# iwanders/spread_spectrum_watermarking

Hardware: AMD Instinct MI355X
Metric: Mpixels/sec embed+extract (4K batch) (higher is better)
Workload: dtype f64

## Files before the change

### spread_spectrum_watermarking_amd/csrc/base_prune.hip

```cpp
#include <algorithm>
#include <cmath>

#include "dct_pair_common.hpp"
#include "dct_pair_colops.hpp"

namespace ssw {

namespace {

constexpr int BP_BINS = 2048;
constexpr int BP_THREADS = 1024;

struct BpKey {
    int ordering;
    float s[2];
    float s0[2];
    float gain;
};

__device__ inline uint32_t bp_sortable(float v) {
    const uint32_t b = __float_as_uint(v);
    return (b & 0x80000000u) ? ~b : (b | 0x80000000u);
}

__global__ __launch_bounds__(BP_THREADS) void base_prune_decide_kernel(const float* __restrict__ coef, const float* __restrict__ energy,
                                                                       unsigned W, unsigned H, BpKey kp, unsigned k,
                                                                       unsigned* __restrict__ need, unsigned long long* __restrict__ stats,
                                                                       double* __restrict__ work, double tile_flop, double tile_bytes,
                                                                       double select_bytes) {
    __shared__ unsigned hist[BP_BINS];
    __shared__ unsigned part[BP_THREADS / 64];
    __shared__ float t_sh;
    __shared__ unsigned any_sh;
    const unsigned tid = threadIdx.x, f = blockIdx.x, tiles = W / SSW_BASE_PRUNE_TILE;
    for (unsigned b = tid; b < BP_BINS; b += BP_THREADS) hist[b] = 0u;
    if (tid == 0) { t_sh = 0.0f; any_sh = 0u; }
    __syncthreads();
    const float* plane = coef + (size_t)f * W * H;
    const unsigned quads = H * (SSW_BASE_PRUNE_TILE / 4);
    for (unsigned q = tid; q < quads; q += BP_THREADS) {
        const unsigned y = q / (SSW_BASE_PRUNE_TILE / 4), x = 4 * (q % (SSW_BASE_PRUNE_TILE / 4));
        const f32x4 c = *reinterpret_cast<const f32x4*>(plane + (size_t)y * W + x);
#pragma unroll
        for (int e = 0; e < 4; ++e) {
            if (y == 0 && x + e == 0) continue;
            float key;
            if (kp.ordering == SSW_ORDER_ENERGY) key = c[e] * c[e];
            else {
                const float scaled = ((x + e) == 0 ? kp.s0[y == 0] : kp.s[y == 0]) * c[e];
                key = scaled * scaled;
            }
            atomicAdd(&hist[bp_sortable(key) >> 21], 1u);
        }
    }
    __syncthreads();
    const unsigned b0 = BP_BINS - 2 - 2 * tid;
    const unsigned h1 = hist[b0 + 1], h0 = hist[b0];
    unsigned v = h1 + h0;
#pragma unroll
    for (int o = 1; o < 64; o <<= 1) {
        const unsigned u = __shfl_up(v, o);
        if ((tid & 63u) >= (unsigned)o) v += u;
    }
    if ((tid & 63u) == 63u) part[tid >> 6] = v;
    __syncthreads();
    unsigned before = 0;
    for (unsigned wv = 0; wv < (tid >> 6); ++wv) before += part[wv];
    const unsigned incl = before + v, excl = incl - h1 - h0;
    if (excl < k && incl >= k) {
        const unsigned bin = excl + h1 >= k ? b0 + 1 : b0;
        const uint32_t sb = (uint32_t)bin << 21;
        t_sh = (sb & 0x80000000u) ? __uint_as_float(sb & 0x7FFFFFFFu) : 0.0f;
    }
    __syncthreads();
    const float T = t_sh;
    const float* e = energy + (size_t)f * W;
    unsigned* nd = need + (size_t)f * tiles;
    for (unsigned t = tid; t < tiles; t += BP_THREADS) nd[t] = t == 0 ? 1u : 0u;
    __syncthreads();
    for (unsigned x = SSW_BASE_PRUNE_TILE + tid; x < W; x += BP_THREADS) {
        const float bound = kp.gain * e[x];
        if (!(T > 1e-30f) || !(bound < T)) { nd[x / SSW_BASE_PRUNE_TILE] = 1u; any_sh = 1u; }
    }
    __syncthreads();
    if (tid == 0 && stats) {
        unsigned computed = 0;
        for (unsigned t = 0; t < tiles; ++t) computed += nd[t];
        if (work) {
            if (computed > 1) {
                atomicAdd(&work[0], (computed - 1) * tile_flop); atomicAdd(&work[1], (computed - 1) * tile_bytes);
                atomicAdd(&work[2], (computed - 1) * select_bytes);
            }
        }
        atomicAdd(&stats[0], (unsigned long long)tiles);
        atomicAdd(&stats[1], (unsigned long long)computed);
        if (any_sh) atomicAdd(&stats[2], 1ull);
    }
}

__global__ __launch_bounds__(256) void base_prune_bound_kernel(const float* __restrict__ energy, unsigned W, size_t total, float gain,
                                                               float* __restrict__ out) {
    const size_t i = blockIdx.x * (size_t)blockDim.x + threadIdx.x;
    if (i >= total) return;
    const size_t f = i / W;
    const unsigned x = (unsigned)(i - f * W), tb = x / SSW_BASE_PRUNE_TILE * SSW_BASE_PRUNE_TILE;
    out[i] = gain * energy[f * W + tb + fwd_cm128_pos(x - tb)];
}

BpKey make_key(size_t w, size_t h, int ordering) {
    float s[2][2];
    select_ortho_scales(w, h, s);
    BpKey kp;
    kp.ordering = ordering;
    kp.s[0] = s[0][0]; kp.s[1] = s[1][0];
    kp.s0[0] = s[0][1]; kp.s0[1] = s[1][1];
    kp.gain = base_prune_gain(w, h, ordering);
    return kp;
}

}

float base_prune_gain(size_t w, size_t h, int ordering) {
    if (ordering != SSW_ORDER_ENERGY && ordering != SSW_ORDER_ENERGY_ORTHOGONAL) return 0.0f;
    if (h == 0 || h >= ((size_t)1 << 17)) return 0.0f;
    double g = 4.0 * (double)h;
    if (ordering == SSW_ORDER_ENERGY_ORTHOGONAL) {
        float s[2][2];
        select_ortho_scales(w, h, s);
        double m = 0.0;
        for (int a = 0; a < 2; ++a) for (int b = 0; b < 2; ++b) m = std::max(m, (double)s[a][b]);
        g *= m * m;
    }
    g *= 1.0 + 1.0 / 32.0;
    return nextafterf((float)g, INFINITY);
}

int launch_base_prune_decide(hipStream_t st, const float* coef, const BasePrune& bp, size_t n_frames, size_t w, size_t h) {
    if (n_frames == 0) return SSW_OK;
    if (!coef || !bp.energy || !bp.need || (reinterpret_cast<uintptr_t>(coef) & 15) != 0 || w % SSW_BASE_PRUNE_TILE != 0 || w > 0xFFFFFFull || h > 0xFFFFFFull || n_frames > 0x7FFFFFFFull ||
        bp.k == 0 || bp.k > 0xFFFFFFFFull) return SSW_ERR_BAD_ARG;
    const BpKey kp = make_key(w, h, bp.ordering);
    if (!(kp.gain > 0.0f)) return SSW_ERR_BAD_ARG;
    base_prune_decide_kernel<<<(unsigned)n_frames, BP_THREADS, 0, st>>>(coef, bp.energy, (unsigned)w, (unsigned)h, kp, (unsigned)bp.k, bp.need,
                                                                       bp.stats, bp.work, bp.tile_flop, bp.tile_bytes, bp.select_bytes);
    SSW_HIP_CHECK(hipGetLastError());
    return SSW_OK;
}

int launch_base_prune_bound(hipStream_t st, const float* energy, size_t n_frames, size_t w, size_t h, int ordering, float* out) {
    const size_t total = n_frames * w;
    if (total == 0) return SSW_OK;
    if (!energy || !out || w % SSW_BASE_PRUNE_TILE != 0) return SSW_ERR_BAD_ARG;
    const float gain = base_prune_gain(w, h, ordering);
    if (!(gain > 0.0f)) return SSW_ERR_UNSUPPORTED;
    base_prune_bound_kernel<<<(unsigned)((total + 255) / 256), 256, 0, st>>>(energy, (unsigned)w, total, gain, out);
    SSW_HIP_CHECK(hipGetLastError());
    return SSW_OK;
}

}
```

### spread_spectrum_watermarking_amd/csrc/dct_pair_f64.hip

```cpp
#include "dct_pair_common.hpp"

#include <cstdlib>
#include <type_traits>

#ifdef SSW_TILE_TRACE
namespace ssw {
__device__ unsigned long long* g_tile_trace = nullptr;
__device__ unsigned int g_tile_trace_cap = 0;
__device__ unsigned int g_tile_trace_n = 0;
__device__ unsigned int* g_tile_kstep = nullptr;
extern "C" int ssw_debug_set_tile_kstep(void* dev_ptr) {
    unsigned int* p = static_cast<unsigned int*>(dev_ptr);
    return hipMemcpyToSymbol(HIP_SYMBOL(g_tile_kstep), &p, sizeof(p)) == hipSuccess ? 0 : -1;
}
extern "C" int ssw_debug_set_tile_trace(void* dev_ptr, unsigned cap) {
    unsigned long long* p = static_cast<unsigned long long*>(dev_ptr);
    unsigned zero = 0;
    if (hipMemcpyToSymbol(HIP_SYMBOL(g_tile_trace), &p, sizeof(p)) != hipSuccess) return -1;
    if (hipMemcpyToSymbol(HIP_SYMBOL(g_tile_trace_cap), &cap, sizeof(cap)) != hipSuccess) return -1;
    if (hipMemcpyToSymbol(HIP_SYMBOL(g_tile_trace_n), &zero, sizeof(zero)) != hipSuccess) return -1;
    return 0;
}
extern "C" int ssw_debug_get_tile_trace_count(unsigned* n) {
    return hipMemcpyFromSymbol(n, HIP_SYMBOL(g_tile_trace_n), sizeof(*n)) == hipSuccess ? 0 : -1;
}
}
#endif
#include "dct_pair_f64_kernel.hpp"
#if defined(SSW_TILE_TRACE) && !defined(SSW_TILE_TRACE_FWD_ONLY)
#define SSW_INV_PART -1
#include "dct_pair_f64_inv.inc"
#endif

namespace ssw {



int launch_dct_pair_gemm_multi_f64(hipStream_t st, bool is_row, bool inverse, int n_classes, const PairClassDesc* desc, float* out,
                                   double* tmp, size_t n_frames, size_t w, size_t h, Epilogue ep, const RgbSink* sink, double* tmp_out,
                                   const PairLayout& lay, const FuseCols* fuse) {
    if (n_frames == 0 || n_classes == 0) return SSW_OK;
    if (n_classes < 0 || n_classes > 8 || !desc) return SSW_ERR_BAD_ARG;
    if (w > 0xFFFFFFull || h > 0xFFFFFFull) return SSW_ERR_BAD_DIMS;
    const bool fuse_rows = fuse && fuse->mode == FUSE_ROWS_COP, fuse_cols = fuse && fuse->mode == FUSE_COLS;
    if (fuse && (!(fuse_rows || fuse_cols) || fuse_rows != is_row || inverse || w % 128 != 0 || h % 16 != 0 ||
                 pair_kpad(h / 8) != dct_pair_fused_units(h))) return SSW_ERR_BAD_ARG;
    if (fuse_rows && (!lay.class_major || sink || !fuse->cop || !fuse->rot1 || !fuse->rot2 || !fuse->rot3)) return SSW_ERR_BAD_ARG;
    const size_t lines = fuse_rows ? n_frames * 16 * dct_pair_fused_units(h) : is_row ? n_frames * h : n_frames * w;
    const size_t len = is_row ? w : h;
    if (lines > 0xFFFFFFFFull) return SSW_ERR_BAD_DIMS;
    const unsigned L = (unsigned)lines;
    const bool with_sink = sink && sink->rgb;
    PairMulti ml;
    PairInstance inst{0, false, 0};
    unsigned tiles_n = 0, leff0 = 0;
    const bool tile48 = tuning(TUNE_TILE48) != 0;
    for (int c = 0; c < n_classes; ++c) {
        PairInstance ic{0, false, 0};
        PairClassArgs& ca = ml.c[c];
        SSW_TRY(pair_class_args(desc[c].cls, is_row, inverse, len, lay, with_sink, tmp_out != nullptr, tile48, ca, ic));
        ca.x1 = desc[c].x1; ca.x2 = desc[c].x2; ca.y1 = desc[c].y1; ca.y2 = desc[c].y2;
        const unsigned ninv = inverse ? (unsigned)(len / pair_class_row(desc[c].cls).inv_ndiv) : 0u;
        if (c == 0) { inst = ic; leff0 = ninv; }
        else if (!(ic == inst) && !(ic.epi == inst.epi && ic.samex == inst.samex && n_classes > 1)) return SSW_ERR_BAD_ARG;
        if (ninv != leff0) return SSW_ERR_BAD_ARG;
        if ((unsigned long long)ml.c[c].Kp * L * 8 > 0xFFFFFFFFull) return SSW_ERR_BAD_DIMS;
        tiles_n += ml.c[c].tiles_n;
    }
    if (n_classes > 1) inst.subname = inverse ? inst.subname : 3;
    const bool small = (unsigned long long)((L + 127) / 128) * tiles_n < 448;
    if (fuse && small) return SSW_ERR_BAD_ARG;
    const int row_part = fuse_rows ? fuse->row_part : 0;
    if (row_part) {
        if ((row_part == 2 && !fuse->need) || (row_part != 1 && row_part != 2)) return SSW_ERR_BAD_ARG;
        tiles_n = 0;
        for (int c = 0; c < n_classes; ++c) {
            PairClassArgs& ca = ml.c[c];
            if (ca.tiles_n < 2 || ca.gsh > 16 || ca.bn32 == 1) return SSW_ERR_BAD_ARG;
            if (row_part == 1) ca.tiles_n = 1;
            else { ca.tn0 = 1; ca.tiles_n -= 1; }
            tiles_n += ca.tiles_n;
        }
    }
    const unsigned BM = small ? 64 : 128;
    if (small)
        for (int c = 0; c < n_classes; ++c)
            if (ml.c[c].bn32 == 2) { tiles_n -= ml.c[c].tiles_n; ml.c[c].bn32 = 0; ml.c[c].tiles_n = (ml.c[c].NP + 63) / 64; tiles_n += ml.c[c].tiles_n; }
    const bool tile0_grid = fuse_cols && fuse->tile_mode == 1;
    const unsigned tiles_m = tile0_grid ? (unsigned)n_frames : (L + BM - 1) / BM;
    if (small && n_classes == 1) {
        const int force = (int)tuning(TUNE_BN32);
        auto balance = [](unsigned long long n) { return (double)n / (256.0 * (double)((n + 255) / 256)); };
        const unsigned tn32 = (ml.c[0].NP + 31) / 32;
        const bool bn32 = force >= 0 ? force != 0 : 0.92 * balance((unsigned long long)tiles_m * tn32) > balance((unsigned long long)tiles_m * tiles_n);
        if (bn32) { ml.c[0].tiles_n = tiles_n = tn32; ml.c[0].bn32 = 1; }
    }
    const unsigned long long nblk = (unsigned long long)tiles_m * tiles_n;
    if (nblk > 0x7FFFFFFFull) return SSW_ERR_BAD_DIMS;
    ml.n_classes = (unsigned)n_classes; ml.L = L; ml.tiles_m = tiles_m; ml.tiles_n_total = tiles_n;
    PairOut po{out, tmp, (unsigned)w, (unsigned)h, (unsigned)(inverse ? leff0 : len), 0, 1, 2};
    po.tmp_out = tmp_out;
    const PairClass c0 = desc[0].cls;
    if (lay.class_major && inverse && pair_class_row(c0).split && c0 != PairClass::R2A) { po.cm = lay.rows_l2 ? 2u : 1u; po.cmt = lay.tile; }
    if (lay.class_major && inverse && c0 == PairClass::R2A) po.cm = 1;
    if (lay.class_major && inverse && is_row && lay.rows_l2 && (c0 == PairClass::E2 || c0 == PairClass::O2)) po.tcm = 1;
    if (lay.class_major && !inverse) po.ft = lay.tile;
    if (fuse_rows) {
        if (inst.samex || inst.epi != EPI_FWD || po.ft != 128) return SSW_ERR_BAD_ARG;
        po.cop = fuse->cop; po.cop_k16 = (unsigned)pair_kpad(h / 8); po.cop_lines = (unsigned)(n_frames * w);
        po.cop_hup = (unsigned)dct_pair_fused_units(h);
        po.crot1 = fuse->rot1; po.crot2 = fuse->rot2; po.crot3 = fuse->rot3;
        inst.epi = EPI_FWD_COLOP;
    }
    if (fuse_cols) po.xperm = 1;
    const bool energy = fuse_rows && fuse->energy != nullptr;
    po.col_energy = energy ? fuse->energy : nullptr;
    ml.need = nullptr; ml.need_mode = 0; ml.need_tpf = 1;
    if (fuse_cols && fuse->tile_mode) {
        if (inst.epi != EPI_FWD || inst.samex || small || (fuse->tile_mode == 2 && !fuse->need)) return SSW_ERR_BAD_ARG;
        ml.need = fuse->need; ml.need_mode = (unsigned)fuse->tile_mode; ml.need_tpf = (unsigned)(w / 128);
    }
    if (row_part == 2) {
        if (energy || po.ft != 128) return SSW_ERR_BAD_ARG;
        ml.need = fuse->need; ml.need_tpf = (unsigned)(w / 128);
        ml.tail = fuse->tail; ml.tail_flop = fuse->tail_flop; ml.tail_bytes = fuse->tail_bytes;
    }
    auto al = [](const void* p, unsigned a) { return (reinterpret_cast<uintptr_t>(p) & (a - 1)) == 0; };
    po.wide = (!is_row && w % 4 == 0 && al(out, 16) && (n_frames * w) % 4 == 0 && (!tmp || al(tmp, 16)) && (!tmp_out || al(tmp_out, 16))) ? 1u : 0u;
    if (with_sink && !(al(sink->iq_i, 16) && al(sink->iq_q, 16) && al(sink->rgb, sink->u8 ? 4 : 16))) po.wide = 0;
    if (with_sink) {
        if (is_row) return SSW_ERR_BAD_ARG;
        po.iq_i = sink->iq_i; po.iq_q = sink->iq_q; po.rgb = sink->rgb; po.rgb_u8 = sink->u8 ? 1u : 0u;
    }
    ml.po = po;
    switch (inst.epi) {
    case EPI_FWD_COLOP:
        if (row_part == 2) SSW_LAUNCH_PAIR_BM(false, EPI_FWD_COLOP, false, 5, 128);
        else if (energy) { if (inst.subname == 4) SSW_LAUNCH_PAIR_BM(false, EPI_FWD_COLOP, false, 14, 128); else SSW_LAUNCH_PAIR_BM(false, EPI_FWD_COLOP, false, 13, 128); }
        else if (inst.subname == 4) SSW_LAUNCH_PAIR_BM(false, EPI_FWD_COLOP, false, 4, 128);
        else SSW_LAUNCH_PAIR_BM(false, EPI_FWD_COLOP, false, 3, 128);
        break;
    case EPI_FWD_ADJ: SSW_LAUNCH_PAIR(false, EPI_FWD_ADJ, false); break;
    case EPI_FWD:
        if (ml.need_mode) SSW_LAUNCH_PAIR_BM(true, EPI_FWD, false, 13, 128);
        else if (inst.subname == 4) SSW_LAUNCH_PAIR_SUB(false, EPI_FWD, false, 4);
        else if (inst.subname == 3) { if (is_row) SSW_LAUNCH_PAIR_SUB(false, EPI_FWD, false, 3); else SSW_LAUNCH_PAIR_SUB(true, EPI_FWD, false, 3); }
        else if (inst.samex) SSW_LAUNCH_ROWCOL(EPI_FWD, true);
        else SSW_LAUNCH_ROWCOL(EPI_FWD, false);
        break;
    default: return launch_pair_gemm_inverse_instances(st, ml, ep, inst, is_row, small, nblk);
    }
    SSW_HIP_CHECK(hipGetLastError());
    return SSW_OK;
}

int launch_dct_pair_gemm_rows_subset_f64(hipStream_t st, const double* x, const double* y, unsigned cap, unsigned Kp, float* out,
                                         unsigned out_stride, unsigned off, size_t lines) {
    if (lines == 0 || cap == 0) return SSW_OK;
    if (lines > 0xFFFFFFFFull || (cap & 1)) return SSW_ERR_BAD_DIMS;
    const unsigned L = (unsigned)lines, NP = cap / 2;
    const unsigned tiles_m = (L + 127) / 128, tiles_n = (NP + 63) / 64;
    const unsigned long long nblk = (unsigned long long)tiles_m * tiles_n;
    if (nblk > 0x7FFFFFFFull) return SSW_ERR_BAD_DIMS;
    if ((unsigned long long)Kp * L * sizeof(double) > 0xFFFFFFFFull) return SSW_ERR_BAD_DIMS;
    PairMulti ml;
    ml.c[0] = PairClassArgs{x, x, y, y + (size_t)NP * 8, NP, Kp, cap, tiles_n, off, off + NP, 1, 0, 0xFFFFFFFFu, 0, 0, 0};
    ml.n_classes = 1; ml.L = L; ml.tiles_m = tiles_m; ml.tiles_n_total = tiles_n;
    ml.po = PairOut{out, nullptr, out_stride, 0, 0, off, off + NP, 1};
    const Epilogue ep{1.f, 1.f};
    pair_gemm_f64_kernel<false, EPI_FWD, true, 2><<<(unsigned)nblk, PT, 0, st>>>(ml, ep);
    SSW_HIP_CHECK(hipGetLastError());
    return SSW_OK;
}

int launch_dct_pair_gemm_rows_subset_split_f64(hipStream_t st, const double* x1, const double* x2, const double* y1, const double* y2,
                                               unsigned cap, unsigned Kp, float* out, unsigned out_stride, unsigned off, size_t lines) {
    if (lines == 0 || cap == 0) return SSW_OK;
    if (lines > 0xFFFFFFFFull) return SSW_ERR_BAD_DIMS;
    const unsigned L = (unsigned)lines, NP = cap;
    const unsigned tiles_m = (L + 127) / 128, tiles_n = (NP + 63) / 64;
    const unsigned long long nblk = (unsigned long long)tiles_m * tiles_n;
    if (nblk > 0x7FFFFFFFull) return SSW_ERR_BAD_DIMS;
    if ((unsigned long long)Kp * L * sizeof(double) > 0xFFFFFFFFull) return SSW_ERR_BAD_DIMS;
    PairMulti ml;
    ml.c[0] = PairClassArgs{x1, x2, y1, y2, NP, Kp, cap, tiles_n, off, 0, 1, 2, 0xFFFFFFFFu, 0, 0, 0};
    ml.n_classes = 1; ml.L = L; ml.tiles_m = tiles_m; ml.tiles_n_total = tiles_n;
    ml.po = PairOut{out, nullptr, out_stride, 0, 0, off, 0, 1};
    const Epilogue ep{1.f, 1.f};
    pair_gemm_f64_kernel<false, EPI_FWD, false, 3><<<(unsigned)nblk, PT, 0, st>>>(ml, ep);
    SSW_HIP_CHECK(hipGetLastError());
    return SSW_OK;
}

int launch_dct_pair_gemm_rows_subset_merged_f64(hipStream_t st, const PairSubsetClass* classes, unsigned n_classes, float* out,
                                                unsigned out_stride, size_t lines) {
    if (lines == 0) return SSW_OK;
    if (lines > 0xFFFFFFFFull) return SSW_ERR_BAD_DIMS;
    const unsigned L = (unsigned)lines, tiles_m = (L + 127) / 128;
    for (int split = 0; split < 2; ++split) {
        PairMulti ml;
        ml.n_classes = 0; ml.L = L; ml.tiles_m = tiles_m; ml.tiles_n_total = 0;
        auto flush = [&]() -> int {
            if (ml.n_classes == 0) return SSW_OK;
            const unsigned long long nblk = (unsigned long long)tiles_m * ml.tiles_n_total;
            if (nblk > 0x7FFFFFFFull) return SSW_ERR_BAD_DIMS;
            ml.po = PairOut{out, nullptr, out_stride, 0, 0, 0, 0, 1};
            const Epilogue ep{1.f, 1.f};
            if (split) pair_gemm_f64_kernel<false, EPI_FWD, false, 3><<<(unsigned)nblk, PT, 0, st>>>(ml, ep);
            else       pair_gemm_f64_kernel<false, EPI_FWD, true, 2><<<(unsigned)nblk, PT, 0, st>>>(ml, ep);
            SSW_HIP_CHECK(hipGetLastError());
            ml.n_classes = 0; ml.tiles_n_total = 0;
            return SSW_OK;
        };
        for (unsigned c = 0; c < n_classes; ++c) {
            const PairSubsetClass& k = classes[c];
            if ((k.x2 != nullptr) != (split != 0) || k.cap == 0) continue;
            if (!split && (k.cap & 1)) return SSW_ERR_BAD_DIMS;
            if ((unsigned long long)k.Kp * L * sizeof(double) > 0xFFFFFFFFull) return SSW_ERR_BAD_DIMS;
            const unsigned NP = split ? k.cap : k.cap / 2, tiles_n = (NP + 63) / 64;
            if (split) ml.c[ml.n_classes] = PairClassArgs{k.x1, k.x2, k.y1, k.y2, NP, k.Kp, k.cap, tiles_n, k.off, 0, 1, 2, 0xFFFFFFFFu, 0, 0, 0};
            else       ml.c[ml.n_classes] = PairClassArgs{k.x1, k.x1, k.y1, k.y1 + (size_t)NP * 8, NP, k.Kp, k.cap, tiles_n, k.off, k.off + NP, 1, 0, 0xFFFFFFFFu, 0, 0, 0};
            ml.tiles_n_total += tiles_n;
            if (++ml.n_classes == 8) SSW_TRY(flush());
        }
        SSW_TRY(flush());
    }
    return SSW_OK;
}

}
```

### spread_spectrum_watermarking_amd/csrc/dct_pair_f64_kernel.hpp

```cpp
#pragma once
#include "dct_pair_common.hpp"
#include "dct_pair_colops.hpp"

#include <cstdlib>
#include <type_traits>


namespace ssw {

constexpr int PT = 256;
constexpr int PBK = 8;
constexpr int RGB_NB = 2;

#ifdef SSW_TILE_TRACE
#define SSW_TT(i) do { if (threadIdx.x == 0) tt[i] = wall_clock64(); } while (0)
#define SSW_KT(t) do { if (threadIdx.x == 0 && (t) < 32u) kst_lds[t] = (unsigned)wall_clock64(); } while (0)
#else
#define SSW_TT(i) do { } while (0)
#define SSW_KT(t) do { } while (0)
#endif
typedef PairOutT<double> PairOut;


struct PairMulti {
    PairClassArgs c[8];
    unsigned n_classes, L, tiles_m, tiles_n_total;
    PairOut po;
    const unsigned* need = nullptr;
    unsigned need_mode = 0, need_tpf = 1;
    unsigned long long* tail = nullptr;
    double tail_flop = 0.0, tail_bytes = 0.0;
};

template <bool COLS, int EPI, bool SAMEX, int SUB = 0, int BM = 128>
__global__ __launch_bounds__(PT, 2) void pair_gemm_f64_kernel(const PairMulti ml, Epilogue ep) {
#if defined(__HIP_DEVICE_COMPILE__)
    constexpr int NX = SAMEX ? 1 : 2;
    constexpr int BN = 64, XQ = BM / 64;
    constexpr int STG = NX * BM * PBK + 2 * BN * PBK;
    constexpr int SXD = 2 * STG;
    constexpr int TRD = COLS ? 4 * 32 * (BM / 2 + 16) / 2 : 0;
#ifdef SSW_TILE_TRACE
    __shared__ __attribute__((aligned(16))) double lds[(SXD > TRD ? SXD : TRD) + 16];
    unsigned* kst_lds = reinterpret_cast<unsigned*>(lds + (SXD > TRD ? SXD : TRD));
#else
    __shared__ __attribute__((aligned(16))) double lds[SXD > TRD ? SXD : TRD];
#endif

#ifdef SSW_TILE_TRACE
    unsigned long long tt[5] = {0, 0, 0, 0, 0};
    const unsigned long long cyc0 = clock64();
    unsigned kslot = 0xFFFFFFFFu;
    if (threadIdx.x == 0 && g_tile_trace) kslot = atomicAdd(&g_tile_trace_n, 1u);
#endif
    SSW_TT(0);
    unsigned tm, tn, cls = 0;
    tile_of_block(blockIdx.x, gridDim.x, ml.tiles_m, ml.tiles_n_total, tm, tn);
    while (cls + 1 < ml.n_classes && tn >= ml.c[cls].tiles_n) { tn -= ml.c[cls].tiles_n; ++cls; }
    if constexpr (COLS && EPI == EPI_FWD && BM == 128 && SUB >= 10) {
        if (ml.need_mode == 1) tm *= ml.need_tpf;
        else if (tm % ml.need_tpf == 0 || ml.need[tm] == 0) return;
    }
    if constexpr (!COLS && EPI == EPI_FWD_COLOP && SUB == 5) {
        const PairClassArgs& cg = ml.c[cls];
        tn += cg.tn0;
        const unsigned tw = cg.bn32 == 2 ? 48u : 64u;
        const unsigned tpf = ml.po.cop_hup / 8, z = tm / tpf;
        const unsigned pf = tn * tw, pl = pf + tw - 1u < cg.NP ? pf + tw - 1u : cg.NP - 1u;
        const unsigned lo = (pf - cg.e2off) >> cg.gsh, hi = pl >> cg.gsh;
        unsigned any = 0;
        for (unsigned t = lo; t <= hi; ++t) any |= ml.need[(size_t)z * ml.need_tpf + t];
        if (!any) return;
        if (ml.tail && tm == z * tpf && threadIdx.x == 0) {
            const double pairs = (double)(pl - pf + 1u);
            atomicAdd(&ml.tail[0], 1ull);
            atomicAdd(reinterpret_cast<double*>(ml.tail) + 1, pairs * ml.tail_flop);
            atomicAdd(reinterpret_cast<double*>(ml.tail) + 2, pairs * ml.tail_bytes);
        }
    }
    const PairClassArgs& ca = ml.c[cls];
    const double* __restrict__ X1g = ca.x1;
    const double* __restrict__ X2g = ca.x2;
    const double* __restrict__ Y1g = ca.y1;
    const double* __restrict__ Y2g = ca.y2;
    const unsigned L = ml.L, NP = ca.NP, Kp = ca.Kp, yrows = ca.yrows;
    PairOut po = ml.po;
    po.c1 = ca.c1; po.c2 = ca.c2; po.cs = ca.cs; po.pm = ca.pm; po.np1 = ca.np1; po.p2lo = ca.p2lo; po.bn32 = ca.bn32; po.fold0 = ca.fold0;
    po.gsh = ca.gsh; po.e2off = ca.e2off;
    const unsigned m0 = tm * BM, p0 = tn * (po.bn32 == 1 ? 32u : po.bn32 == 2 ? 48u : (unsigned)BN);
    const unsigned tid = threadIdx.x;
    const unsigned lane = tid & 63, wave = tid >> 6;
    const unsigned li = lane & 15, lq = lane >> 4;

    const unsigned wv = (unsigned)__builtin_amdgcn_readfirstlane((int)wave);
    const unsigned drow = 16 * wave + (lane >> 2), dch = lane & 3;
    unsigned xoff[XQ];
#pragma unroll
    for (int q = 0; q < XQ; ++q) {
        const unsigned j = drow + 64 * q;
        unsigned r = m0 + ((COLS && BM == 128 && po.xperm) ? fwd_cm128_pos(j) : j);
        r = r < L ? r : L - 1;
        xoff[q] = (r - m0) * 64u + 16u * (dch ^ ((j >> 2) & 3u));
    }
    unsigned yr = p0 + drow;
    yr = yr < NP ? yr : NP - 1;
    const unsigned yoff = (yr - p0) * 64u + 16u * (dch ^ ((drow >> 2) & 3u));
#ifdef SSW_ABL_X0
    const size_t m0x = 0;
#else
    const size_t m0x = m0;
#endif
    const __amdgpu_buffer_rsrc_t x1r = __builtin_amdgcn_make_buffer_rsrc((void*)(X1g + m0x * 8), 0, 0xFFFFFFFFu, 0x00020000);
    const __amdgpu_buffer_rsrc_t x2r = __builtin_amdgcn_make_buffer_rsrc((void*)(X2g + m0x * 8), 0, 0xFFFFFFFFu, 0x00020000);
    const __amdgpu_buffer_rsrc_t y1r = __builtin_amdgcn_make_buffer_rsrc((void*)(Y1g + (size_t)p0 * 8), 0, 0xFFFFFFFFu, 0x00020000);
    const __amdgpu_buffer_rsrc_t y2r = __builtin_amdgcn_make_buffer_rsrc((void*)(Y2g + (size_t)p0 * 8), 0, 0xFFFFFFFFu, 0x00020000);
    const unsigned xstep = L * 64u, ystep = yrows * 64u;

    constexpr int LPT = XQ * NX + 2;
    typedef __attribute__((address_space(3))) void* lds_ptr_t;
    auto issue = [&](unsigned t, unsigned sb) {
        const unsigned xadv = t * xstep, yadv = t * ystep;
        double* b = lds + sb + 16 * wv * PBK;
#pragma unroll
        for (int q = 0; q < XQ; ++q) {
            __builtin_amdgcn_raw_ptr_buffer_load_lds(x1r, (lds_ptr_t)(b + 64 * q * PBK), 16, xoff[q], xadv, 0, 0);
            if (!SAMEX) __builtin_amdgcn_raw_ptr_buffer_load_lds(x2r, (lds_ptr_t)(b + BM * PBK + 64 * q * PBK), 16, xoff[q], xadv, 0, 0);
        }
        __builtin_amdgcn_raw_ptr_buffer_load_lds(y1r, (lds_ptr_t)(b + NX * BM * PBK), 16, yoff, yadv, 0, 0);
        __builtin_amdgcn_raw_ptr_buffer_load_lds(y2r, (lds_ptr_t)(b + NX * BM * PBK + BN * PBK), 16, yoff, yadv, 0, 0);
    };
    auto run = [&](auto nic, auto njc) {
    constexpr int NI = decltype(nic)::value;
    constexpr int NJ = decltype(njc)::value;
    constexpr int NJA = NJ < 2 ? 2 : NJ;
    constexpr bool FULL = NI == BM / 32;
    const unsigned wm = FULL ? (wave >> 1) * (BM / 2) : wave * (BM / 4), wn = FULL ? (wave & 1) * 32 : 0;
    f64x4 acc1[NI][NJA], acc2[NI][NJA];
#pragma unroll
    for (int i = 0; i < NI; ++i)
#pragma unroll
        for (int j = 0; j < NJA; ++j) { acc1[i][j] = (f64x4){0, 0, 0, 0}; acc2[i][j] = (f64x4){0, 0, 0, 0}; }

    const unsigned fsw = (li >> 2) & 3;
    unsigned rdx[2], rdy[2];
#pragma unroll
    for (int sh = 0; sh < 2; ++sh) {
        rdx[sh] = (wm + li) * PBK + 2 * ((2 * sh + (lq >> 1)) ^ fsw) + (lq & 1);
        rdy[sh] = NX * BM * PBK + (wn + li) * PBK + 2 * ((2 * sh + (lq >> 1)) ^ fsw) + (lq & 1);
    }
    struct Frag { double x1[NI], x2[NI], y1[NJA], y2[NJA]; };
    auto fread = [&](unsigned sb, auto shc, Frag& f) {
        constexpr int sh = decltype(shc)::value;
        const double* b = lds + sb;
#pragma unroll
        for (int jn = 0; jn < NJ; ++jn) {
            f.y1[jn] = b[rdy[sh] + 16 * jn * PBK];
            f.y2[jn] = b[rdy[sh] + BN * PBK + 16 * jn * PBK];
        }
#pragma unroll
        for (int i = 0; i < NI; ++i) {
            f.x1[i] = b[rdx[sh] + 16 * i * PBK];
            if (!SAMEX) f.x2[i] = b[rdx[sh] + BM * PBK + 16 * i * PBK];
        }
    };
    auto fmma = [&](const Frag& f) {
#pragma unroll
        for (int i = 0; i < NI; ++i)
#pragma unroll
            for (int jn = 0; jn < NJ; ++jn) {
                const double xb = SAMEX ? f.x1[i] : f.x2[i];
                if (!COLS) {
                    acc1[i][jn] = __builtin_amdgcn_mfma_f64_16x16x4f64(f.x1[i], f.y1[jn], acc1[i][jn], 0, 0, 0);
                    acc2[i][jn] = __builtin_amdgcn_mfma_f64_16x16x4f64(xb, f.y2[jn], acc2[i][jn], 0, 0, 0);
                } else {
                    acc1[i][jn] = __builtin_amdgcn_mfma_f64_16x16x4f64(f.y1[jn], f.x1[i], acc1[i][jn], 0, 0, 0);
                    acc2[i][jn] = __builtin_amdgcn_mfma_f64_16x16x4f64(f.y2[jn], xb, acc2[i][jn], 0, 0, 0);
                }
            }
    };
    using B0 = std::integral_constant<int, 0>;
    using B1 = std::integral_constant<int, 1>;
    auto interleave = [&](auto dmac) {
        constexpr int NDMA = decltype(dmac)::value;
        constexpr int NMF = 2 * NJ * NI;
        constexpr int NRD = (2 * NJ + NI * NX + 1) / 2;
#pragma unroll
        for (int i = 0; i < NRD; ++i) {
            __builtin_amdgcn_sched_group_barrier(0x008, 1, 0);
            __builtin_amdgcn_sched_group_barrier(0x100, 1, 0);
        }
#pragma unroll
        for (int i = 0; i < NDMA; ++i) {
            __builtin_amdgcn_sched_group_barrier(0x008, 1, 0);
            __builtin_amdgcn_sched_group_barrier(0x020, 1, 0);
        }
        __builtin_amdgcn_sched_group_barrier(0x008, NMF - NRD - NDMA > 0 ? NMF - NRD - NDMA : 0, 0);
        __builtin_amdgcn_sched_barrier(0);
    };
    const unsigned nk = Kp / PBK;
    Frag fa, fb;
    issue(0, 0);
    issue(1, STG);
    asm volatile("s_waitcnt vmcnt(%0)" :: "n"(LPT) : "memory");
    asm volatile("s_barrier" ::: "memory");
    SSW_TT(1);
    fread(0u, B0{}, fa);
    unsigned cur = 0, nxt = STG, t = 0;
    auto step = [&](auto issuec) {
        constexpr bool ISSUE = decltype(issuec)::value != 0;
        fread(cur, B1{}, fb);
        fmma(fa);
        interleave(B0{});
        asm volatile("s_waitcnt vmcnt(0) lgkmcnt(0)\n\ts_barrier" ::: "memory");
// ... 597 lines not shown
                        const unsigned ln = m0 + wm + 16 * i + li;
                        const unsigned lz = ln < L ? ln / W : 0, lc = ln < L ? ln - lz * W : 0;
                        const double* tp = po.tmp + (size_t)lz * (n / 2) * W + lc;
#pragma unroll
                        for (int r = 0; r < 4; ++r) {
                            const unsigned pair = p0 + wn + 16 * jn + lq + 4 * r;
                            const unsigned pc = pair < NP ? pair : 0;
                            const unsigned nn = half ? po.c2 + po.cs * p2(pc) : po.c1 + po.cs * pc;
                            e[i][r] = tp[(size_t)(nn < n / 2 ? nn : 0) * W];
                        }
                    }
                    (void)tpl;
                    lds_order();
#pragma unroll
                    for (int i = 0; i < NI; ++i)
#pragma unroll
                        for (int r = 0; r < 4; ++r) {
                            const double a = half ? acc2[i][jn][r] : acc1[i][jn][r];
                            tw[wr0 + (4 * r) * TPF + 16 * i] = (float)(e[i][r] + a);
                            tw[wr0 + (16 + 4 * r) * TPF + 16 * i] = (float)(e[i][r] - a);
                        }
                    lds_order();
                    if constexpr (EPI == EPI_INV_O_RGB) {
                        if (rgb_fast) {
                            auto rgb_round = [&](auto u8c) {
                            constexpr bool U8 = decltype(u8c)::value;
                            constexpr int NB = NRI < RGB_NB ? NRI : RGB_NB;
#pragma unroll
                            for (int tb = 0; tb < NRI; tb += NB) {
                                unsigned off[NB];
                                float fac[NB];
                                f32x4 v[NB], iv[NB], qv[NB];
#pragma unroll
                                for (int u = 0; u < NB; ++u) {
                                    const int t = tb + u;
                                    const unsigned srow = t * RPI + rrow;
                                    const unsigned pair = p0 + wn + 16 * jn + (srow & 15);
                                    v[u] = *reinterpret_cast<const f32x4*>(trd + t * RPI * TPF);
                                    const unsigned pc = pair < NP ? pair : 0;
                                    const unsigned nn = half ? po.c2 + po.cs * p2(pc) : po.c1 + po.cs * pc;
                                    const bool ok = line_ok && pair < NP && nn < n / 2;
                                    const unsigned idx = srow < 16 ? nn : n - 1 - nn;
                                    off[u] = ok ? idx * W + col : 0x20000000u;
                                    fac[u] = idx == 0 ? ep.first : ep.base;
                                    iv[u] = __builtin_bit_cast(f32x4, __builtin_amdgcn_raw_buffer_load_b128(rgb_i, off[u] * 4u, 0, 0));
                                    qv[u] = __builtin_bit_cast(f32x4, __builtin_amdgcn_raw_buffer_load_b128(rgb_q, off[u] * 4u, 0, 0));
                                }
#pragma unroll
                                for (int u = 0; u < NB; ++u) {
                                    float y[4], c[12];
#pragma unroll
                                    for (int e4 = 0; e4 < 4; ++e4) y[e4] = plain ? v[u][e4] : v[u][e4] * fac[u];
                                    pair_rgb_of_quad(y, iv[u], qv[u], c);
                                    if (U8) {
                                        unsigned w3[3];
                                        pair_rgb8_words(c, w3);
                                        __builtin_amdgcn_raw_buffer_store_b96((u32x3){w3[0], w3[1], w3[2]}, rgb_o, off[u] * 3u, 0, 0);
                                    } else {
#pragma unroll
                                        for (int d = 0; d < 3; ++d)
                                            __builtin_amdgcn_raw_buffer_store_b128(__builtin_bit_cast(u32x4, (f32x4){c[4 * d], c[4 * d + 1], c[4 * d + 2], c[4 * d + 3]}),
                                                                                   rgb_o, off[u] * 12u + 16u * d, 0, 0);
                                    }
                                }
                            }
                            };
                            if (po.rgb_u8) rgb_round(std::true_type{}); else rgb_round(std::false_type{});
                            continue;
                        }
                    }
#pragma unroll
                    for (int t = 0; t < NRI; ++t) {
                        const unsigned srow = t * RPI + rrow;
                        const unsigned pair = p0 + wn + 16 * jn + (srow & 15);
                        const f32x4 v = *reinterpret_cast<const f32x4*>(trd + t * RPI * TPF);
                        if (!line_ok || pair >= NP) continue;
                        const unsigned nn = half ? po.c2 + po.cs * p2(pair) : po.c1 + po.cs * pair;
                        if (nn >= n / 2) continue;
                        put_quad(srow < 16 ? nn : n - 1 - nn, v);
                    }
                }
        }
        trace_end();
        return;
      }
    }
    if constexpr (COLS) {
#pragma unroll
        for (int i = 0; i < NI; ++i) {
            const unsigned line = m0 + wm + 16 * i + li;
            if (line >= L) continue;
            const unsigned z = line / W, col = line - z * W;
            float* lp = po.out + (size_t)z * H * W + col;
            double* tp = po.tmp + (size_t)z * (n / 2) * W + col;
            if (EPI == EPI_INV_O_RGB) {
                const size_t base = (size_t)z * H * W + col;
#pragma unroll
                for (int jn = 0; jn < NJ; ++jn)
#pragma unroll
                    for (int r = 0; r < 4; r += 2) {
                        double e1[2], e2[2];
                        bool ok1[2], ok2[2];
                        unsigned m1[2], m2[2];
#pragma unroll
                        for (int q = 0; q < 2; ++q) {
                            const unsigned pair = p0 + wn + 16 * jn + lq + 4 * (r + q);
                            const unsigned pc = pair < NP ? pair : 0;
                            const unsigned n1 = po.c1 + po.cs * pc, n2 = po.c2 + po.cs * p2(pc);
                            ok1[q] = pair < NP && n1 < n / 2;
                            ok2[q] = pair < NP && n2 < n / 2;
                            m1[q] = ok1[q] ? n1 : 0;
                            m2[q] = ok2[q] ? n2 : 0;
                            e1[q] = tp[(size_t)m1[q] * W];
                            e2[q] = tp[(size_t)m2[q] * W];
                        }
#pragma unroll
                        for (int q = 0; q < 2; ++q) {
                            const double a1 = acc1[i][jn][r + q], a2 = acc2[i][jn][r + q];
                            const unsigned idx1[2] = {m1[q], n - 1 - m1[q]}, idx2[2] = {m2[q], n - 1 - m2[q]};
                            const float v1[2] = {(float)(e1[q] + a1), (float)(e1[q] - a1)}, v2[2] = {(float)(e2[q] + a2), (float)(e2[q] - a2)};
                            unsigned px1[2], px2[2];
                            float y1[2], y2[2];
#pragma unroll
                            for (int o = 0; o < 2; ++o) {
                                px1[o] = idx1[o] * W; y1[o] = apply_epilogue(ep, v1[o], idx1[o]);
                                px2[o] = idx2[o] * W; y2[o] = apply_epilogue(ep, v2[o], idx2[o]);
                            }
                            pair_store_rgb_batch<double, 2>(po, base, px1, y1, ok1[q]);
                            pair_store_rgb_batch<double, 2>(po, base, px2, y2, ok2[q]);
                        }
                    }
                continue;
            }
#pragma unroll
            for (int jn = 0; jn < NJ; ++jn)
#pragma unroll
                for (int r = 0; r < 4; ++r) {
                    const unsigned pair = p0 + wn + 16 * jn + lq + 4 * r;
                    if (pair >= NP) continue;
                    emit(lp, tp, po.tmp_out + (size_t)z * n * W + col, W, pair, acc1[i][jn][r], acc2[i][jn][r]);
                }
        }
    }
    trace_end();
    };
    using J1 = std::integral_constant<int, 1>;
    using J2 = std::integral_constant<int, 2>;
    using J3 = std::integral_constant<int, 3>;
    const bool j3 = BM == 128 && (po.bn32 == 2 || (!COLS && NP - p0 <= 48));
    if (NP - p0 <= 16 && po.bn32 != 2) run(std::integral_constant<int, BM / 64>{}, J1{});
    else if (po.bn32 != 2 && (NP - p0 <= 32 || po.bn32)) run(std::integral_constant<int, BM / 64>{}, J2{});
    else if (j3)                       run(std::integral_constant<int, BM / 64>{}, J3{});
    else                               run(std::integral_constant<int, BM / 32>{}, J2{});
#endif
}

#define SSW_LAUNCH_PAIR_BM(COLS, EPI, SAMEX, SUBV, BMV) \
        pair_gemm_f64_kernel<COLS, EPI, SAMEX, SUBV, BMV><<<(unsigned)nblk, PT, 0, st>>>(ml, ep)
#define SSW_LAUNCH_PAIR_SUB(COLS, EPI, SAMEX, SUBV) do { if (small) SSW_LAUNCH_PAIR_BM(COLS, EPI, SAMEX, SUBV, 64); else SSW_LAUNCH_PAIR_BM(COLS, EPI, SAMEX, SUBV, 128); } while (0)
#define SSW_LAUNCH_PAIR(COLS, EPI, SAMEX) do { if (inst.subname == 0) SSW_LAUNCH_PAIR_SUB(COLS, EPI, SAMEX, 0); else SSW_LAUNCH_PAIR_SUB(COLS, EPI, SAMEX, 1); } while (0)
#define SSW_LAUNCH_ROWCOL(EPI, SAMEX) do { if (is_row) SSW_LAUNCH_PAIR(false, EPI, SAMEX); else SSW_LAUNCH_PAIR(true, EPI, SAMEX); } while (0)

int launch_pair_gemm_inverse_instances(hipStream_t st, const PairMulti& ml, Epilogue ep, const PairInstance& inst, bool is_row, bool small,
                                       unsigned long long nblk);

}
```

### spread_spectrum_watermarking_amd/csrc/ssw_internal.hpp

```cpp
#pragma once

#include <hip/hip_runtime.h>

#include <cstddef>
#include <cstdint>
#include <functional>
#include <map>
#include <string>
#include <tuple>
#include <utility>
#include <vector>

#include "../../include/ssw.h"
#include "dct_plan.hpp"
#include "dct_pair_class.hpp"

namespace ssw {

void set_last_error(const std::string& s);

#define SSW_HIP_CHECK(expr)                                                              \
    do {                                                                                 \
        hipError_t e__ = (expr);                                                         \
        if (e__ != hipSuccess) {                                                         \
            ::ssw::set_last_error(std::string(#expr) + ": " + hipGetErrorString(e__));   \
            return (e__ == hipErrorOutOfMemory) ? SSW_ERR_OUT_OF_MEMORY : SSW_ERR_HIP;   \
        }                                                                                \
    } while (0)

#define SSW_TRY(expr)                         \
    do {                                      \
        int s__ = (expr);                     \
        if (s__ != SSW_OK) return s__;        \
    } while (0)


int launch_rgb_to_yiq(hipStream_t st, const float* rgb, size_t npix, float* y, float* i, float* q);
int launch_yiq_to_rgb(hipStream_t st, const float* y, const float* i, const float* q, size_t npix,
                      float* rgb);
int launch_synth(hipStream_t st, uint32_t seed, uint32_t first_frame, size_t n_frames, size_t w,
                 size_t h, float* rgb);

size_t dense_basis_kpad(size_t n);
int launch_make_basis_f32(hipStream_t st, size_t n, bool inverse, float* out);
int launch_make_basis_f64(hipStream_t st, size_t n, bool inverse, double* out);

struct Epilogue {
    float first, base;
};
int launch_dct_rows(hipStream_t st, int precision, const float* in, float* out, size_t rows, size_t w,
                    const void* basis, Epilogue ep);
int launch_dct_cols(hipStream_t st, int precision, const float* in, float* out, size_t n_frames,
                    size_t w, size_t h, const void* basis, Epilogue ep);
int launch_dct_rows_f64out(hipStream_t st, const float* in, double* out, size_t rows, size_t w, const double* basis);
int launch_dct_cols_f64out(hipStream_t st, const float* in, double* out, size_t n_frames, size_t w, size_t h, const double* basis);

size_t dct_pair_kpad(size_t n);
size_t dct_pair_operand_elems(size_t n_frames, size_t w, size_t h);
int launch_make_half_basis_blocked(hipStream_t st, size_t n, bool inverse, int parity, double* out);
int launch_dct_pair_prep(hipStream_t st, bool is_row, bool inverse, const float* in, size_t n_frames, size_t w, size_t h,
                         double* o1, double* o2);
enum class PixFmt { F32, U8, U16 };
constexpr size_t pix_bytes(PixFmt f) { return f == PixFmt::U8 ? 1 : f == PixFmt::U16 ? 2 : 4; }
constexpr unsigned pix_align_mask(PixFmt f) { return f == PixFmt::U8 ? 3u : f == PixFmt::U16 ? 7u : 15u; }
bool dct_pair_can_prep_from_rgb(size_t w, size_t h, const void* rgb, PixFmt fmt);
enum class RowSrc { Plane, RgbF32, RgbU8, RgbU16 };
constexpr RowSrc row_src(PixFmt f) { return f == PixFmt::U8 ? RowSrc::RgbU8 : f == PixFmt::U16 ? RowSrc::RgbU16 : RowSrc::RgbF32; }
constexpr PixFmt pix_fmt(RowSrc s) { return s == RowSrc::RgbU8 ? PixFmt::U8 : s == RowSrc::RgbU16 ? PixFmt::U16 : PixFmt::F32; }
struct RowInput {
    RowSrc kind; const void* p; float *i, *q;
    static RowInput plane(const float* y) { return {RowSrc::Plane, y, nullptr, nullptr}; }
    static RowInput rgb(PixFmt f, const void* frames, float* i = nullptr, float* q = nullptr) { return {row_src(f), frames, i, q}; }
};
int launch_dct_pair_prep4(hipStream_t st, bool is_row, bool inverse, const RowInput& in, size_t n_frames, size_t w, size_t h,
                          double* q1, double* q2, double* p);
int launch_dct_pair_prep8_rows(hipStream_t st, const RowInput& in, size_t n_frames, size_t w, size_t h,
                               double* r1, double* r2, double* m, double* p);
struct RgbSink {
    const float* iq_i = nullptr;
    const float* iq_q = nullptr;
    void* rgb = nullptr;
    bool u8 = false;
};
int launch_dct_pair_prep8_cols(hipStream_t st, const float* in, size_t n_frames, size_t w, size_t h,
                               double* r1, double* r2, double* m, double* p);
enum { FUSE_ROWS_COP = 1, FUSE_COLS = 2 };
struct FuseCols {
    int mode = 0; double* cop = nullptr; const double *rot1 = nullptr, *rot2 = nullptr, *rot3 = nullptr;
    float* energy = nullptr;
    const unsigned* need = nullptr;
    int tile_mode = 0;
    int row_part = 0;
    unsigned long long* tail = nullptr;
    double tail_flop = 0.0, tail_bytes = 0.0;
};
struct PairClassDesc { PairClass cls; const double *x1, *x2, *y1, *y2; };
int launch_dct_pair_gemm_multi_f64(hipStream_t st, bool is_row, bool inverse, int n_classes, const PairClassDesc* desc, float* out,
                                   double* tmp, size_t n_frames, size_t w, size_t h, Epilogue ep, const RgbSink* sink = nullptr,
                                   double* tmp_out = nullptr, const PairLayout& layout = PairLayout(), const FuseCols* fuse = nullptr);

int launch_dct_pair_gemm_rows_subset_f64(hipStream_t st, const double* x, const double* y, unsigned cap, unsigned Kp, float* out,
                                         unsigned out_stride, unsigned off, size_t lines);
int launch_dct_pair_gemm_rows_subset_split_f64(hipStream_t st, const double* x1, const double* x2, const double* y1, const double* y2,
                                               unsigned cap, unsigned Kp, float* out, unsigned out_stride, unsigned off, size_t lines);
struct PairSubsetClass {
    const double *x1, *x2, *y1, *y2;
    unsigned cap, Kp, off;
};
int launch_dct_pair_gemm_rows_subset_merged_f64(hipStream_t st, const PairSubsetClass* classes, unsigned n_classes, float* out,
                                                unsigned out_stride, size_t lines);
size_t dct_pair_split_kpad(size_t len);
enum { TUNE_EFOLD_MIN, TUNE_EFOLD_INV_MIN, TUNE_EFOLD_COLS_MIN, TUNE_CLASS_TILE, TUNE_DEEP_MIN_ROWS, TUNE_DEEP_MIN_COLS, TUNE_PREP_STAGED,
       TUNE_MERGE_MAX_LINES, TUNE_BN32, TUNE_BAND_SPLIT, TUNE_FUSE_COLS, TUNE_UPLOAD_BANDS, TUNE_SPECULATE_K, TUNE_PREP_LIGHT, TUNE_LANE_STAGGER, TUNE_DERIVED_FUSED, TUNE_TILE48, TUNE_BASE_PRUNE, TUNE_BASE_ENERGY_LOWP, TUNE_COUNT };
long long tuning(int which);
int launch_prep16_cols_l2(hipStream_t st, const float* in, size_t n_frames, size_t w, size_t h, double* base,
                          const double* rot1, const double* rot2, const double* rot3, bool class_major, bool in_l2, unsigned K16);
int launch_prep16_inv_cols_l2(hipStream_t st, const float* in, size_t n_frames, size_t w, size_t h, double* base,
                              const double* rot1, const double* rot2, const double* rot3, bool class_major, bool in_l2, unsigned K16);
int launch_prep16_cols_staged(hipStream_t st, const float* in, size_t n_frames, size_t w, size_t h, double* base,
                              const double* rot1, const double* rot2, bool class_major, bool semi, unsigned K8, unsigned K16, bool efold);
int launch_prep16_inv_cols_staged(hipStream_t st, const float* in, size_t n_frames, size_t w, size_t h, double* base,
                                  const double* rot1, const double* rot2, bool class_major, bool semi, unsigned K8, unsigned K16, bool l2);
int launch_prep16_inv_rows_l2(hipStream_t st, const float* in, size_t rows, size_t w, double* base,
                              const double* rot1, const double* rot2, const double* rot3, unsigned K16);
int launch_prep16_inv_rows_staged(hipStream_t st, const float* in, size_t rows, size_t w, double* base,
                                  const double* rot1, const double* rot2, unsigned K8, unsigned K16);
size_t dct_pair_split_elems(size_t n_frames, size_t w, size_t h);
size_t dct_pair_split_basis_rows(size_t len, int which);
int launch_make_split_basis_blocked(hipStream_t st, size_t n, bool inverse, int which, double* out);
int launch_make_rot_table(hipStream_t st, size_t n, double* out);
int launch_dct_pair_rotate(hipStream_t st, const double* p, const double* rot, double* sp, size_t lines, size_t len);
size_t dct_pair_semi_deep_elems(size_t lines, size_t len);
int launch_dct_pair_prep16_inv_rows(hipStream_t st, const float* in, size_t n_frames, size_t w, size_t h, double* base,
                                    const double* rot1, const double* rot2, const double* rot3, PrepFamily prep);
int launch_dct_pair_prep16_inv_cols(hipStream_t st, const float* in, size_t n_frames, size_t w, size_t h, double* base,
                                    const double* rot1, const double* rot2, const double* rot3, PrepFamily prep, const PairLayout& lay);
int launch_dct_pair_prep16_cols(hipStream_t st, const float* in, size_t n_frames, size_t w, size_t h, double* base,
                                const double* rot1, const double* rot2, const double* rot3, PrepFamily prep, const PairLayout& lay);
size_t dct_pair_deep_elems(size_t lines, size_t len);
int launch_dct_pair_prep16_rows(hipStream_t st, const RowInput& in, size_t n_frames, size_t w, size_t h, double* base,
                                const double* rot1, const double* rot2, const double* rot3, bool l2, bool unit_order = false);
inline size_t dct_pair_fused_units(size_t h) { return ((h / 16 + 7) / 8) * 8; }

constexpr unsigned PRUNE_NO_REM = 0xFFFFFFFFu;
constexpr uint32_t PRUNE_NEG = 0x40000000u;
constexpr unsigned SSW_PRUNE_INFO = 16;
struct PruneClass { unsigned mod, rem, cap, off, rem2 = PRUNE_NO_REM, radd = 0; };
struct PrunePlan {
    unsigned n_classes = 0;
    PruneClass c[9];
    unsigned W = 0, cap_total = 0;
};
static_assert(SSW_PRUNE_INFO >= 1 + sizeof(PrunePlan::c) / sizeof(PruneClass), "a chunk's info block holds the flag and one count per class");
int launch_prune_build(hipStream_t st, const uint32_t* idx, size_t n_frames, size_t k, const PrunePlan& plan,
                       uint32_t* flag , uint32_t* rows , uint32_t* pos , uint32_t* info );
struct PruneGatherJob {
    const uint32_t* rows;
    const char* src;
    char* dst;
    unsigned cap, src_rows, kblocks, first_block;
    bool negate;
    bool frag = false;
};
struct PruneGatherJobs {
    PruneGatherJob j[18];
    unsigned n;
};
int launch_prune_gather_bases(hipStream_t st, PruneGatherJobs jobs);
int launch_extract_pruned(hipStream_t st, const float* base, const float* compact, size_t n_frames, size_t w, size_t h,
                          size_t cap, const uint32_t* pos, const uint32_t* indices, size_t k, int method, float alpha,
                          float* out);

constexpr unsigned SSW_BASE_PRUNE_TILE = 128;
constexpr unsigned SSW_BASE_PRUNE_STATS = 16;
struct BasePrune {
    float* energy = nullptr;
    unsigned* need = nullptr;
    unsigned long long* stats = nullptr;
    size_t k = 0;
    int ordering = 0;
    double* work = nullptr;
    double tile_flop = 0.0, tile_bytes = 0.0, select_bytes = 0.0;
    bool* decided = nullptr;
    std::function<int(hipStream_t)>* tail = nullptr;
};
float base_prune_gain(size_t w, size_t h, int ordering);
int launch_base_prune_decide(hipStream_t st, const float* coef, const BasePrune& bp, size_t n_frames, size_t w, size_t h);
int launch_base_prune_bound(hipStream_t st, const float* energy, size_t n_frames, size_t w, size_t h, int ordering, float* out);

struct BaseEnergyClass {
    const double *x1 = nullptr, *x2 = nullptr;
    const void* y16 = nullptr;
    unsigned NP = 0, Kp = 0, pair0 = 0, pm = 0, c1 = 0, c2 = 0, gsh = 0, e2off = 0;
};
size_t base_energy_split_bytes(unsigned NP, unsigned Kp, unsigned pair0);
int launch_base_energy_split(hipStream_t st, const double* y1, const double* y2, unsigned yrows, unsigned NP, unsigned Kp, unsigned pair0, void* out);
int launch_base_energy_bound(hipStream_t st, int n_classes, const BaseEnergyClass* cls, size_t n_frames, size_t w, size_t h, size_t lines_per_frame,
                             float factor, float* energy);

struct SelectWorkspace {
    uint32_t* hist = nullptr;
    uint32_t* ctrl = nullptr;
    uint64_t* cand = nullptr;
    size_t frames = 0, cap = 0;
    uint32_t* fallbacks = nullptr;
};
size_t select_cand_capacity(size_t k);
size_t select_max_k();
void select_ortho_scales(size_t w, size_t h, float s[2][2]);
int launch_topk(hipStream_t st, const float* coef, size_t n_frames, size_t w, size_t h, int ordering,
                size_t k, const SelectWorkspace& ws, uint32_t* indices, const unsigned* need = nullptr, unsigned need_tile = 0,
                size_t cand_cap = 0);
struct ResizeTaps {
    uint32_t max_taps = 0;
    std::vector<uint32_t> left, count;
    std::vector<float> weights;
};
struct DeviceTaps {
    uint32_t* left = nullptr;
    uint32_t* count = nullptr;
    float* weights = nullptr;
    uint32_t max_taps = 0;
    uint32_t span[8] = {0};
    bool quad_uniform = false;
};
void build_resize_taps(size_t in_len, size_t out_len, ResizeTaps& t);
int launch_u8_to_f32(hipStream_t st, const uint8_t* in, size_t n, float* out);
int launch_f32_to_u8(hipStream_t st, const float* in, size_t n, uint8_t* out);
int launch_rgb8_to_yiq(hipStream_t st, const uint8_t* rgb, size_t npix, float* y, float* i, float* q);
int launch_u16_to_f32(hipStream_t st, const uint16_t* in, size_t n, float* out);
int launch_f32_to_u16(hipStream_t st, const float* in, size_t n, uint16_t* out);
int launch_rgb16_to_yiq(hipStream_t st, const uint16_t* rgb, size_t npix, float* y, float* i, float* q);
int launch_yiq_to_rgb8(hipStream_t st, const float* y, const float* i, const float* q, size_t npix, uint8_t* rgb);
size_t resize_tmp_bytes(const uint8_t* in, size_t n_frames, size_t w, size_t h, size_t nw, size_t nh, const DeviceTaps& vt,
                        const DeviceTaps& ht, const uint8_t* out);
int launch_resize_rgb8(hipStream_t st, const uint8_t* in, size_t n_frames, size_t w, size_t h, size_t nw, size_t nh,
                       const DeviceTaps& vt, const DeviceTaps& ht, float* tmp, uint8_t* out);

int full_sort_scratch_bytes(size_t plane_len, size_t n_frames, size_t* bytes);
int launch_full_sort(hipStream_t st, const float* coef, size_t n_frames, size_t w, size_t h, int ordering, void* scratch,
                     size_t scratch_bytes, uint32_t* indices_out, size_t k);
int launch_embed(hipStream_t st, float* coef, size_t n_frames, size_t plane_len,
                 const uint32_t* indices, size_t idx_stride, const float* marks,
                 const uint32_t* mark_offsets, const uint32_t* mark_lens, size_t n_marks,
                 size_t max_len, size_t mark_stride , int method, float alpha);
int launch_extract(hipStream_t st, const float* base, const float* derived, size_t n_frames,
                   size_t plane_len, const uint32_t* indices, size_t k, int method, float alpha,
                   float* out);
int launch_similarity(hipStream_t st, const float* extracted, const float* marks, size_t n_pairs,
                      size_t k, float* sims);
int launch_extract_shared(hipStream_t st, const float* base, const float* derived, size_t n_frames, size_t plane_len,
                          const uint32_t* indices, size_t k, int method, float alpha, float* out);
int launch_extract_shared_pruned(hipStream_t st, const float* base, const float* compact, size_t n_frames, size_t w, size_t h,
                                 size_t cap, const uint32_t* pos, const uint32_t* indices, size_t k, int method, float alpha,
                                 float* out);
int launch_trace_finish(hipStream_t st, const float* sims, size_t n_rows, size_t n_marks, float threshold, const float* extracted,
                        const float* marks, size_t k, uint32_t* best, float* best_sim, uint32_t* n_exceed);
int launch_gemm_nt_f32(hipStream_t st, const float* A, size_t M, const float* B, size_t N, size_t K, float* out);
int launch_sim_den(hipStream_t st, const float* extracted, size_t n_ext, size_t k, float* den);
int launch_sim_scale(hipStream_t st, float* sims, const float* den, size_t n_ext, size_t n_marks);
int launch_widen_indices(hipStream_t st, const uint32_t* in, size_t n, uint64_t* out);

}

namespace ssw { namespace host { struct Transfer; } }

struct ssw_ctx {
    int device = 0;
    hipStream_t stream = nullptr;
    hipStream_t own_stream = nullptr;
    size_t chunk_frames = 0;

    std::map<std::tuple<size_t, bool, bool, ssw::BasisKind>, void*> basis;
    std::map<std::tuple<size_t, int, unsigned>, void*> split16;
    bool fold = true;
    int fold_level = SSW_DCT_FOLDING_DEFAULT;

    struct Buf {
        void* p = nullptr;
        size_t bytes = 0;
    };
    struct Lane {
        Buf plane[4];
        Buf operand[6];
        Buf idx;
        ssw::SelectWorkspace sel;
        Buf compact[2];
        Buf gathered;
        Buf prune_u32;
        Buf base_prune;
        hipStream_t cur = nullptr;
        hipEvent_t done = nullptr;
    };
    static constexpr int MAX_LANES = 2;
    Lane lane[MAX_LANES];
    hipStream_t aux_stream = nullptr;
    bool overlap = true;
    bool prune = true;
    bool split = true;
    std::vector<hipEvent_t> sync_events;
    size_t sync_next = 0;
    Buf overflow;
    uint64_t pruned_chunks = 0, redone_chunks = 0;
    uint64_t pruned_columns = 0;
    Buf base_prune_stats;
    double base_prune_billed[5] = {0.0, 0.0, 0.0, 0.0, 0.0};
    hipStream_t copy_stream = nullptr;
    struct FrameStage {
        Buf buf;
        static constexpr int MAX_BANDS = 4;
        hipEvent_t uploaded[MAX_BANDS] = {nullptr, nullptr, nullptr, nullptr};
        hipEvent_t consumed = nullptr;
        bool in_use = false;
    };
    FrameStage frame_stage[2];
    unsigned frame_stage_next = 0;
    size_t expected_k = 0;
    std::multimap<size_t, void*> plane_pool;
    size_t plane_pool_bytes = 0;
    struct RgbSpare { void* p; size_t bytes; hipEvent_t released; };
    std::vector<RgbSpare> rgb_spares;
    std::vector<void*> retired;
    uint32_t* select_fallbacks = nullptr;
    uint64_t select_frames = 0;
    ssw::host::Transfer* xfer = nullptr;
    hipStream_t down_stream = nullptr;
    struct HostStream {
        static constexpr int NB = 3;
        Buf in[NB], in2[NB], out[NB];
        Buf marks, ext, sims;
        hipEvent_t up_done[NB] = {}, k_done[NB] = {}, down_done[NB] = {};
        bool active = false;
    };
    HostStream hs;
    Buf small;
    Buf sort_scratch;
    Buf resize_tmp;
    Buf restore_base;
    Buf trace[6];
    Buf locate[6];
    Buf catalogue[3];
    Buf jpeg;
    Buf filter;
    Buf fingerprint[6];
    std::map<std::pair<size_t, size_t>, ssw::DeviceTaps> taps;

    bool timing = false;
    double stage_ms[SSW_STAGE_COUNT] = {0};
    uint64_t stage_launches[SSW_STAGE_COUNT] = {0};
    double stage_bytes[SSW_STAGE_COUNT] = {0};
    double stage_work[SSW_STAGE_COUNT] = {0};
    struct Pending {
        int stage;
        hipEvent_t a, b;
        int alias = -1;
    };
    std::vector<Pending> pending;
    std::vector<hipEvent_t> free_events;
    hipEvent_t tail_event = nullptr;
    hipStream_t tail_stream = nullptr;
    bool tail_fresh = false;
};
namespace ssw { inline PlanSettings plan_settings(const ssw_ctx* ctx) { return PlanSettings{ctx->fold, ctx->fold_level, ctx->split}; } }
```

### spread_spectrum_watermarking_amd/csrc/ssw_lib.hip

```cpp
#include <algorithm>
#include <cmath>
#include <cstdlib>
#include <cstring>
#include <new>

#include "resize_common.hpp"
#include "ssw_host.hpp"

namespace ssw {
static thread_local std::string g_last_error;
void set_last_error(const std::string& s) { g_last_error = s; }
}

using namespace ssw;
using namespace ssw::host;

struct ssw_writer {
    ssw_ctx* ctx;
    size_t w, h;
    ssw_config cfg;
    float *y = nullptr, *i = nullptr, *q = nullptr;
    float* y0 = nullptr;
    uint32_t* idx = nullptr;
    size_t idx_k = 0;
// ... 102 lines not shown
    {
        ssw_ctx::FrameStage& fs = ctx->frame_stage[ctx->frame_stage_next & 1];
        SSW_TRY(grow(fs.buf, bytes));
        const bool no_split = tuning(TUNE_BAND_SPLIT) == 0;
        long long nb = tuning(TUNE_UPLOAD_BANDS);
        nb = nb < 2 ? 2 : nb > ssw_ctx::FrameStage::MAX_BANDS ? ssw_ctx::FrameStage::MAX_BANDS : nb;
        while (nb > 2 && ((bytes / nb) % 16 != 0 || !can_split_forward_rows(ctx, precision == SSW_PRECISION_F64, w, h, (size_t)nb, y, tmp, fs.buf.p, fmt))) --nb;
        if (!no_split && bytes >= ((size_t)8 << 20) &&
            can_split_forward_rows(ctx, precision == SSW_PRECISION_F64, w, h, (size_t)nb, y, tmp, fs.buf.p, fmt)) {
            ++ctx->frame_stage_next;
            SSW_TRY(frame_stage_events(fs));
            if (fs.in_use) SSW_HIP_CHECK(hipStreamWaitEvent(ctx->copy_stream, fs.consumed, 0));
            const size_t hb = bytes / nb, hp = plane / nb, rows = h / nb;
            bool in_flight = false;
            int rc = SSW_OK;
            for (int band = 0; band < (int)nb && rc == SSW_OK; ++band) {
                bool async = false;
                rc = upload_nowait(ctx, (char*)fs.buf.p + band * hb, (const char*)host_rgb + band * hb, hb, ctx->copy_stream, &async);
                in_flight = in_flight || async;
                if (rc == SSW_OK && hipEventRecord(fs.uploaded[band], ctx->copy_stream) != hipSuccess) rc = SSW_ERR_HIP;
                if (rc == SSW_OK && hipStreamWaitEvent(ctx->stream, fs.uploaded[band], 0) != hipSuccess) rc = SSW_ERR_HIP;
                untimed_work(ctx);
                if (rc != SSW_OK) break;
                Chain ch;
                rc = build_forward_rows_band(ctx, ctx->lane[0], precision, (char*)fs.buf.p + band * hb, fmt, w, rows, h, tmp + band * hp,
                                             i ? i + band * hp : nullptr, q ? q + band * hp : nullptr, ch);
                if (rc == SSW_OK) rc = run_serial(ch, ctx->stream);
            }
            if (rc == SSW_OK) rc = stage_consumed(ctx, fs);
            if (rc == SSW_OK) {
                Chain ch;
                rc = build_forward_cols_after_rows(ctx, ctx->lane[0], precision, w, h, tmp, y, ch);
                if (rc == SSW_OK) rc = run_serial(ch, ctx->stream);
            }
            if (in_flight && hipStreamSynchronize(ctx->copy_stream) != hipSuccess && rc == SSW_OK) rc = SSW_ERR_HIP;
            return rc;
        }
    }
    ssw_ctx::FrameStage* fs = nullptr;
    SSW_TRY(stage_frame_in(ctx, host_rgb, bytes, &fs));
    Chain ch;
    SSW_TRY(build_forward_from_rgb(ctx, ctx->lane[0], precision, fs->buf.p, fmt, 1, w, h, y, i, q, tmp, ch));
    SSW_TRY(run_serial(ch, ctx->stream));
    return stage_consumed(ctx, *fs);
}
int similarity_matrix_enqueue(ssw_ctx* ctx, const float* dev_extracted, size_t n_extracted, const float* dev_marks, size_t n_marks,
                              size_t k, float* dev_sims) {
    SSW_TRY(grow(ctx->small, n_extracted * sizeof(float)));
    StageTimer t(ctx, SSW_STAGE_SIMILARITY, ctx->stream);
    SSW_TRY(launch_sim_den(ctx->stream, dev_extracted, n_extracted, k, (float*)ctx->small.p));
    SSW_TRY(launch_gemm_nt_f32(ctx->stream, dev_extracted, n_extracted, dev_marks, n_marks, k, dev_sims));
    return launch_sim_scale(ctx->stream, dev_sims, (const float*)ctx->small.p, n_extracted, n_marks);
}
}

namespace ssw {
namespace host {
int trace_check_args(const ssw_ctx* ctx, const ssw_config* cfg, size_t w, size_t h, size_t k, const void* marks, size_t n_marks,
                     const void* sims, const void* best, const void* best_sim, const void* n_exceed) {
    if (!ctx) return SSW_ERR_BAD_ARG;
    if (!marks && (n_marks || sims || best || best_sim || n_exceed)) return SSW_ERR_BAD_ARG;
    SSW_TRY(check_config(cfg));
    if (w == 0 || h == 0) return SSW_ERR_BAD_DIMS;
    if (k >= w * h) return SSW_ERR_K_TOO_LARGE;
    return SSW_OK;
}

int trace_score(ssw_ctx* ctx, const float* dev_extracted, size_t n_suspects, const float* dev_marks, size_t n_marks, size_t k,
                float threshold, float* dev_sims, uint32_t* dev_best, float* dev_best_sim, uint32_t* dev_n_exceed) {
    if (n_suspects == 0 || (!dev_sims && !dev_best && !dev_best_sim && !dev_n_exceed)) return SSW_OK;
    float* sims = dev_sims;
    if (!sims && n_marks) {
        SSW_TRY(grow(ctx->trace[5], n_suspects * n_marks * sizeof(float)));
        sims = (float*)ctx->trace[5].p;
    }
    if (n_marks && k) SSW_TRY(similarity_matrix_enqueue(ctx, dev_extracted, n_suspects, dev_marks, n_marks, k, sims));
    else if (n_marks) { SSW_HIP_CHECK(hipMemsetAsync(sims, 0xFF, n_suspects * n_marks * sizeof(float), ctx->stream)); untimed_work(ctx); }
    StageTimer t(ctx, SSW_STAGE_SIMILARITY, ctx->stream);
    return launch_trace_finish(ctx->stream, sims, n_suspects, k ? n_marks : 0, threshold, dev_extracted, dev_marks, k, dev_best, dev_best_sim,
                               dev_n_exceed);
}
}
}

namespace {
int fingerprint_trace_impl(ssw_ctx* ctx, const ssw_config* cfg, const void* dev_base_rgb, const void* dev_suspect_rgb, PixFmt fmt,
                           size_t n_suspects, size_t w, size_t h, size_t k, const float* dev_marks, size_t n_marks, float threshold,
                           float* dev_extracted, float* dev_sims, uint32_t* dev_best, float* dev_best_sim, uint32_t* dev_n_exceed) {
    if (!ctx || !dev_base_rgb || !dev_suspect_rgb || !dev_extracted) return SSW_ERR_BAD_ARG;
    SSW_TRY(trace_check_args(ctx, cfg, w, h, k, dev_marks, n_marks, dev_sims, dev_best, dev_best_sim, dev_n_exceed));
    if (n_suspects == 0) return SSW_OK;
    CtxGuard g(ctx);
    const float* yb = nullptr;
    const uint32_t* idx = nullptr;
    SSW_TRY(trace_base(ctx, *cfg, dev_base_rgb, fmt, w, h, k, &yb, &idx));
    SSW_TRY(trace_extract(ctx, *cfg, yb, idx, dev_suspect_rgb, fmt, n_suspects, w, h, k, dev_extracted));
    return trace_score(ctx, dev_extracted, n_suspects, dev_marks, n_marks, k, threshold, dev_sims, dev_best, dev_best_sim, dev_n_exceed);
}
}

extern "C" {

const char* ssw_version(void) { return "ssw-hip 0.1.0 (gfx950)"; }
int ssw_build_all_strategies(void) { return 0; }

int ssw_ctx_transform_plan(ssw_ctx* ctx, size_t n_frames, size_t w, size_t h, int dct_type, uint32_t* flags) {
    if (!ctx || !flags || w == 0 || h == 0) return SSW_ERR_BAD_ARG;
    const ssw::PlanSettings s = ssw::plan_settings(ctx);
    *flags = ssw::plan_flags(ssw::plan_transform({dct_type, SSW_PRECISION_F64, std::min(n_frames, ssw::plan_frame_limit(s, true, w, h)), w, h,
                                                  0, false, true, s}));
    return SSW_OK;
}

const char* ssw_status_string(int s) {
    switch (s) {
    case SSW_OK: return "ok";
    case SSW_ERR_BAD_ARG: return "bad argument";
    case SSW_ERR_BAD_DIMS: return "bad dimensions";
    case SSW_ERR_LENGTH_MISMATCH: return "Derived coefficient length not equal to base coefficient length.";
    case SSW_ERR_K_TOO_LARGE: return "Desired extraction length exceeds available coefficients.";
    case SSW_ERR_NOT_BASE: return "reader was not created as a base reader";
    case SSW_ERR_UNSUPPORTED: return "unsupported (custom closures cannot run on the device)";
    case SSW_ERR_CONSUMED: return "writer already consumed";
    case SSW_ERR_HIP: return "HIP runtime error";
    case SSW_ERR_NO_DEVICE: return "no HIP device (this library has no CPU path)";
    case SSW_ERR_OUT_OF_MEMORY: return "out of device memory";
    default: return "unknown status";
    }
}

const char* ssw_last_error(void) { return g_last_error.c_str(); }

void ssw_config_default(ssw_config* cfg) {
    if (!cfg) return;
    cfg->ordering = SSW_ORDER_ENERGY;
    cfg->method = SSW_OPTION2;
    cfg->alpha = 0.1f;
    cfg->precision = SSW_PRECISION_F64;
}

int ssw_ctx_create(int device_id, ssw_ctx** out) {
    if (!out) return SSW_ERR_BAD_ARG;
    *out = nullptr;
    int count = 0;
    if (hipGetDeviceCount(&count) != hipSuccess || count <= 0) {
        set_last_error("hipGetDeviceCount: no device");
        return SSW_ERR_NO_DEVICE;
    }
    if (device_id < 0 || device_id >= count) return SSW_ERR_BAD_ARG;
    DeviceGuard g(device_id);
    ssw_ctx* ctx = new (std::nothrow) ssw_ctx();
    if (!ctx) return SSW_ERR_OUT_OF_MEMORY;
    ctx->device = device_id;
    hipError_t e = hipStreamCreateWithFlags(&ctx->own_stream, hipStreamNonBlocking);
    if (e != hipSuccess) { delete ctx; set_last_error(hipGetErrorString(e)); return SSW_ERR_HIP; }
    ctx->stream = ctx->own_stream;
    e = hipStreamCreateWithFlags(&ctx->aux_stream, hipStreamNonBlocking);
    if (e != hipSuccess) { (void)hipStreamDestroy(ctx->own_stream); delete ctx; set_last_error(hipGetErrorString(e)); return SSW_ERR_HIP; }
    e = hipStreamCreateWithFlags(&ctx->copy_stream, hipStreamNonBlocking);
    if (e != hipSuccess) {
        (void)hipStreamDestroy(ctx->aux_stream); (void)hipStreamDestroy(ctx->own_stream);
        delete ctx; set_last_error(hipGetErrorString(e)); return SSW_ERR_HIP;
    }
    if (hipMalloc((void**)&ctx->select_fallbacks, sizeof(uint32_t)) != hipSuccess ||
        hipMemset(ctx->select_fallbacks, 0, sizeof(uint32_t)) != hipSuccess) {
        (void)hipGetLastError();
        if (ctx->select_fallbacks) (void)hipFree(ctx->select_fallbacks);
        (void)hipStreamDestroy(ctx->copy_stream); (void)hipStreamDestroy(ctx->aux_stream); (void)hipStreamDestroy(ctx->own_stream);
        delete ctx; set_last_error("hipMalloc: selection counter"); return SSW_ERR_OUT_OF_MEMORY;
    }
    const char* ov = std::getenv("SSW_OVERLAP");
    if (ov) ctx->overlap = std::atoi(ov) != 0;
    const char* pr = std::getenv("SSW_PRUNE");
    if (pr) ctx->prune = std::atoi(pr) != 0;
    const char* sp = std::getenv("SSW_ODD_SPLIT");
    if (sp) ctx->split = std::atoi(sp) != 0;
    *out = ctx;
    return SSW_OK;
}

int ssw_ctx_destroy(ssw_ctx* ctx) {
    if (!ctx) return SSW_OK;
    CtxGuard g(ctx);
    (void)hipStreamSynchronize(ctx->stream);
    if (ctx->aux_stream) (void)hipStreamSynchronize(ctx->aux_stream);
    if (ctx->copy_stream) (void)hipStreamSynchronize(ctx->copy_stream);
    if (ctx->down_stream) (void)hipStreamSynchronize(ctx->down_stream);
    transfer_destroy(ctx);
    for (int s = 0; s < ssw_ctx::HostStream::NB; ++s) {
        release(ctx->hs.in[s]); release(ctx->hs.in2[s]); release(ctx->hs.out[s]);
        for (hipEvent_t e : {ctx->hs.up_done[s], ctx->hs.k_done[s], ctx->hs.down_done[s]}) if (e) (void)hipEventDestroy(e);
    }
    release(ctx->hs.marks); release(ctx->hs.ext); release(ctx->hs.sims);
    for (void* p : ctx->retired) (void)hipFree(p);
    ctx->retired.clear();
    (void)plane_pool_flush(ctx);
    for (auto& fs : ctx->frame_stage) {
        release(fs.buf);
        for (hipEvent_t e : fs.uploaded)
            if (e) (void)hipEventDestroy(e);
        if (fs.consumed) (void)hipEventDestroy(fs.consumed);
    }
    for (auto& kv : ctx->basis) (void)hipFree(kv.second);
    for (auto& kv : ctx->split16) (void)hipFree(kv.second);
    for (auto& ln : ctx->lane) {
        for (auto& b : ln.plane) release(b);
        for (auto& b : ln.operand) release(b);
        for (auto& b : ln.compact) release(b);
        release(ln.idx);
        release(ln.gathered);
        release(ln.prune_u32);
        release(ln.base_prune);
        release_select(ln.sel);
    }
    if (ctx->select_fallbacks) (void)hipFree(ctx->select_fallbacks);
    release(ctx->overflow);
    release(ctx->base_prune_stats);
    release(ctx->small);
    release(ctx->sort_scratch);
    release(ctx->resize_tmp);
    release(ctx->restore_base);
    for (auto& b : ctx->fingerprint) release(b);
    for (auto& b : ctx->trace) release(b);
    for (auto& b : ctx->locate) release(b);
    for (auto& b : ctx->catalogue) release(b);
    release(ctx->jpeg);
    release(ctx->filter);
    for (auto& kv : ctx->taps) { (void)hipFree(kv.second.left); (void)hipFree(kv.second.count); (void)hipFree(kv.second.weights); }
    for (auto& e : ctx->sync_events) (void)hipEventDestroy(e);
    for (auto& p : ctx->pending) { (void)hipEventDestroy(p.a); (void)hipEventDestroy(p.b); }
    for (auto& e : ctx->free_events) (void)hipEventDestroy(e);
    if (ctx->aux_stream) (void)hipStreamDestroy(ctx->aux_stream);
    if (ctx->copy_stream) (void)hipStreamDestroy(ctx->copy_stream);
    if (ctx->down_stream) (void)hipStreamDestroy(ctx->down_stream);
    (void)hipStreamDestroy(ctx->own_stream);
    delete ctx;
    return SSW_OK;
}

int ssw_ctx_synchronize(ssw_ctx* ctx) {
    if (!ctx) return SSW_ERR_BAD_ARG;
    CtxGuard g(ctx);
    SSW_HIP_CHECK(hipStreamSynchronize(ctx->stream));
    return SSW_OK;
}

void* ssw_ctx_stream(ssw_ctx* ctx) { return ctx ? (void*)ctx->stream : nullptr; }

int ssw_ctx_set_stream(ssw_ctx* ctx, void* hip_stream) {
    if (!ctx) return SSW_ERR_BAD_ARG;
    CtxGuard g(ctx);
    SSW_TRY(flush_timers(ctx));
    SSW_HIP_CHECK(hipStreamSynchronize(ctx->stream));
    ctx->stream = hip_stream ? (hipStream_t)hip_stream : ctx->own_stream;
    return SSW_OK;
}

int ssw_ctx_wait_event(ssw_ctx* ctx, void* hip_event) {
    if (!ctx || !hip_event) return SSW_ERR_BAD_ARG;
    CtxGuard g(ctx);
    SSW_HIP_CHECK(hipStreamWaitEvent(ctx->stream, (hipEvent_t)hip_event, 0));
    return SSW_OK;
}

int ssw_ctx_record_event(ssw_ctx* ctx, void* hip_event) {
    if (!ctx || !hip_event) return SSW_ERR_BAD_ARG;
    CtxGuard g(ctx);
    SSW_HIP_CHECK(hipEventRecord((hipEvent_t)hip_event, ctx->stream));
    return SSW_OK;
}

int ssw_ctx_set_chunk_frames(ssw_ctx* ctx, size_t frames) {
    if (!ctx) return SSW_ERR_BAD_ARG;
    ctx->chunk_frames = frames;
    return SSW_OK;
}

size_t ssw_ctx_pass_frames(ssw_ctx* ctx, size_t n_frames, size_t w, size_t h) {
    return ctx ? effective_chunk(ctx, w, h, n_frames) : 0;
}

int ssw_ctx_set_dct_folding(ssw_ctx* ctx, int enable) {
    if (!ctx) return SSW_ERR_BAD_ARG;
    if (enable < 0 || enable > 6) return SSW_ERR_BAD_ARG;
    ctx->fold = enable != 0;
    ctx->fold_level = enable;
    return SSW_OK;
}

int ssw_ctx_enable_timing(ssw_ctx* ctx, int enable) {
    if (!ctx) return SSW_ERR_BAD_ARG;
    CtxGuard g(ctx);
    SSW_TRY(flush_timers(ctx));
    ctx->timing = enable != 0;
    return SSW_OK;
}

int ssw_ctx_reset_timing(ssw_ctx* ctx) {
    if (!ctx) return SSW_ERR_BAD_ARG;
    CtxGuard g(ctx);
    SSW_TRY(flush_timers(ctx));
    for (int s = 0; s < SSW_STAGE_COUNT; ++s) { ctx->stage_ms[s] = 0; ctx->stage_launches[s] = 0; ctx->stage_work[s] = 0; ctx->stage_bytes[s] = 0; }
    ctx->pruned_chunks = ctx->redone_chunks = ctx->pruned_columns = 0;
    ctx->select_frames = 0;
    SSW_HIP_CHECK(hipStreamSynchronize(ctx->stream));
    if (ctx->aux_stream) SSW_HIP_CHECK(hipStreamSynchronize(ctx->aux_stream));
    SSW_HIP_CHECK(hipMemset(ctx->select_fallbacks, 0, sizeof(uint32_t)));
// ... 889 lines not shown
```

### spread_spectrum_watermarking_amd/csrc/ssw_pipeline.hip

```cpp
#include <algorithm>
#include <cmath>
#include <cstring>

#include "ssw_host.hpp"
#include "dct_pair_split.hpp"

#include <array>
#include <cstdlib>

namespace ssw {
namespace host {

namespace { thread_local ssw_ctx* tl_ctx = nullptr; }
CtxGuard::CtxGuard(ssw_ctx* ctx) : dg(ctx->device), prev(tl_ctx) {
    tl_ctx = ctx;
    if (prev != ctx) { ctx->tail_event = nullptr; ctx->tail_fresh = false; }
    if (prev != ctx && !ctx->retired.empty()) {
        for (void* p : ctx->retired) (void)hipFree(p);
        ctx->retired.clear();
    }
}
CtxGuard::~CtxGuard() { tl_ctx = prev; }

size_t plane_pool_flush(ssw_ctx* ctx) {
    size_t bytes = ctx->plane_pool_bytes;
    for (auto& kv : ctx->plane_pool) (void)hipFree(kv.second);
    ctx->plane_pool.clear();
    ctx->plane_pool_bytes = 0;
    for (auto& sp : ctx->rgb_spares) { (void)hipFree(sp.p); (void)hipEventDestroy(sp.released); bytes += sp.bytes; }
    ctx->rgb_spares.clear();
    return bytes;
}

size_t host_stream_release(ssw_ctx* ctx) {
    ssw_ctx::HostStream& hs = ctx->hs;
    if (hs.active) return 0;
    size_t bytes = 0;
    for (int s = 0; s < ssw_ctx::HostStream::NB; ++s)
        for (ssw_ctx::Buf* b : {&hs.in[s], &hs.in2[s], &hs.out[s]})
            if (b->p) { bytes += b->bytes; (void)hipFree(b->p); b->p = nullptr; b->bytes = 0; }
    return bytes;
}

int dev_malloc(void** p, size_t bytes) {
    *p = nullptr;
    hipError_t e = hipMalloc(p, bytes ? bytes : 16);
    if (e == hipSuccess) return SSW_OK;
    (void)hipGetLastError();
    if (tl_ctx && (!tl_ctx->plane_pool.empty() || !tl_ctx->rgb_spares.empty())) {
        (void)plane_pool_flush(tl_ctx);
        e = hipMalloc(p, bytes ? bytes : 16);
        if (e == hipSuccess) return SSW_OK;
        (void)hipGetLastError();
    }
    if (tl_ctx && host_stream_release(tl_ctx)) {
        e = hipMalloc(p, bytes ? bytes : 16);
        if (e == hipSuccess) return SSW_OK;
        (void)hipGetLastError();
    }
    *p = nullptr;
    set_last_error(std::string("hipMalloc(") + std::to_string(bytes) + " bytes): " + hipGetErrorString(e));
    return SSW_ERR_OUT_OF_MEMORY;
}

int grow(ssw_ctx::Buf& b, size_t bytes) {
    if (b.bytes >= bytes && b.p) return SSW_OK;
    if (b.p) {
        if (tl_ctx) tl_ctx->retired.push_back(b.p);
        else SSW_HIP_CHECK(hipFree(b.p));
        b.p = nullptr; b.bytes = 0;
    }
    SSW_ALLOC(&b.p, bytes);
    b.bytes = bytes ? bytes : 16;
    return SSW_OK;
}

void release(ssw_ctx::Buf& b) {
    if (b.p) (void)hipFree(b.p);
    b.p = nullptr;
    b.bytes = 0;
}

void release_select(SelectWorkspace& s) {
    if (s.hist) (void)hipFree(s.hist);
    if (s.ctrl) (void)hipFree(s.ctrl);
    if (s.cand) (void)hipFree(s.cand);
    s = SelectWorkspace();
}

int grow_select(hipStream_t st, SelectWorkspace& s, size_t frames, size_t k) {
    const size_t want = select_cand_capacity(k);
    if (s.frames >= frames && s.cap >= want && s.hist) return SSW_OK;
    const size_t nf = std::max(frames, s.frames), cap = std::max(want, s.cap);
    release_select(s);
    SSW_ALLOC(&s.hist, nf * 2048 * sizeof(uint32_t));
    SSW_ALLOC(&s.ctrl, nf * 4 * sizeof(uint32_t));
    SSW_ALLOC(&s.cand, nf * cap * sizeof(uint64_t));
    SSW_HIP_CHECK(hipMemsetAsync(s.hist, 0, nf * 2048 * sizeof(uint32_t), st));
    SSW_HIP_CHECK(hipMemsetAsync(s.ctrl, 0, nf * 4 * sizeof(uint32_t), st));
    untimed_work(tl_ctx);
    s.frames = nf;
    s.cap = cap;
    return SSW_OK;
}

static hipEvent_t timer_event(ssw_ctx* ctx, hipStream_t st) {
    if (ctx->tail_event && ctx->tail_fresh && ctx->tail_stream == st) return ctx->tail_event;
    hipEvent_t e = nullptr;
    if (!ctx->free_events.empty()) { e = ctx->free_events.back(); ctx->free_events.pop_back(); }
    else if (hipEventCreateWithFlags(&e, hipEventReleaseToDevice) != hipSuccess) return nullptr;
    if (hipEventRecord(e, st) != hipSuccess) { ctx->free_events.push_back(e); return nullptr; }
    ctx->tail_event = e; ctx->tail_stream = st; ctx->tail_fresh = true;
    return e;
}
StageTimer::StageTimer(ssw_ctx* c, int s, hipStream_t stream, double work, int alias_stage) : ctx(c), stage(s), st(stream), alias(alias_stage) {
    if (!ctx->timing) return;
    ctx->stage_work[stage] += work;
    if (alias >= 0) ctx->stage_work[alias] += work;
    const bool gemm = stage == SSW_STAGE_DCT_ROW || stage == SSW_STAGE_DCT_COL || stage == SSW_STAGE_DCT_ROW_MAIN || stage == SSW_STAGE_DCT_COL_MAIN;
    if (!gemm) ctx->stage_bytes[stage] += work;
    a = timer_event(ctx, st);
    ctx->tail_fresh = false;
    armed = a != nullptr;
}
void StageTimer::traffic(double bytes) {
    if (ctx->timing) ctx->stage_bytes[stage] += bytes;
}
StageTimer::~StageTimer() {
    if (!ctx->timing || !armed) return;
    b = timer_event(ctx, st);
    if (b) ctx->pending.push_back({stage, a, b, alias});
}

int flush_timers(ssw_ctx* ctx) {
    std::vector<hipEvent_t> used;
    for (auto& p : ctx->pending) {
        float ms = 0.f;
        SSW_HIP_CHECK(hipEventSynchronize(p.b));
        SSW_HIP_CHECK(hipEventElapsedTime(&ms, p.a, p.b));
        ctx->stage_ms[p.stage] += ms;
        ctx->stage_launches[p.stage] += 1;
        if (p.alias >= 0) { ctx->stage_ms[p.alias] += ms; ctx->stage_launches[p.alias] += 1; }
        used.push_back(p.a);
        used.push_back(p.b);
    }
    ctx->pending.clear();
    std::sort(used.begin(), used.end());
    used.erase(std::unique(used.begin(), used.end()), used.end());
    for (hipEvent_t e : used) ctx->free_events.push_back(e);
    ctx->tail_event = nullptr; ctx->tail_fresh = false;
    if (ctx->base_prune_stats.p) {
        double wk[3] = {0.0, 0.0, 0.0};
        SSW_HIP_CHECK(hipMemcpy(wk, (const char*)ctx->base_prune_stats.p + 4 * sizeof(unsigned long long), sizeof(wk), hipMemcpyDeviceToHost));
        if (ctx->timing) {
            ctx->stage_work[SSW_STAGE_DCT_COL] += wk[0] - ctx->base_prune_billed[0];
            ctx->stage_bytes[SSW_STAGE_DCT_COL] += wk[1] - ctx->base_prune_billed[1];
            ctx->stage_work[SSW_STAGE_SELECT] += wk[2] - ctx->base_prune_billed[2];
            ctx->stage_bytes[SSW_STAGE_SELECT] += wk[2] - ctx->base_prune_billed[2];
        }
        for (int i = 0; i < 3; ++i) ctx->base_prune_billed[i] = wk[i];
        double tw[2] = {0.0, 0.0};
        SSW_HIP_CHECK(hipMemcpy(tw, (const char*)ctx->base_prune_stats.p + 9 * sizeof(unsigned long long), sizeof(tw), hipMemcpyDeviceToHost));
        if (ctx->timing) {
            ctx->stage_work[SSW_STAGE_DCT_ROW] += tw[0] - ctx->base_prune_billed[3];
            ctx->stage_bytes[SSW_STAGE_DCT_ROW] += tw[1] - ctx->base_prune_billed[4];
        }
        for (int i = 0; i < 2; ++i) ctx->base_prune_billed[3 + i] = tw[i];
    }
    return SSW_OK;
}

int get_basis(ssw_ctx* ctx, size_t n, bool inverse, bool f64, BasisKind kind, const void** out) {
    typedef BasisKind B;
    auto key = std::make_tuple(n, inverse, f64, kind);
    auto it = ctx->basis.find(key);
    if (it != ctx->basis.end()) { *out = it->second; return SSW_OK; }
    void* p = nullptr;
    if (kind != B::Dense && !f64) return SSW_ERR_BAD_ARG;
    const bool half = kind == B::HalfEven || kind == B::HalfOdd, rot = kind == B::Rot;
    const int split_which = kind == B::SinELaunch ? 4 : (int)kind - (int)B::CosE;
    const size_t elems = kind == B::Dense ? n * dense_basis_kpad(n)
                       : rot  ? n / 2
                       : half ? (n / 2) * dct_pair_kpad(n)
                              : dct_pair_split_basis_rows(n, split_which) * dct_pair_split_kpad(n);
    SSW_ALLOC(&p, std::max<size_t>(elems, 1) * (f64 ? sizeof(double) : sizeof(float)));
    int rc = rot  ? launch_make_rot_table(ctx->stream, n, (double*)p)
             : half ? launch_make_half_basis_blocked(ctx->stream, n, inverse, kind == B::HalfOdd ? 1 : 0, (double*)p)
             : kind != B::Dense ? launch_make_split_basis_blocked(ctx->stream, n, inverse, split_which, (double*)p)
             : f64  ? launch_make_basis_f64(ctx->stream, n, inverse, (double*)p)
                    : launch_make_basis_f32(ctx->stream, n, inverse, (float*)p);
    untimed_work(ctx);
    if (rc != SSW_OK) { (void)hipFree(p); return rc; }
    ctx->basis[key] = p;
    *out = p;
    return SSW_OK;
}

int get_split16(ssw_ctx* ctx, size_t len, PairClass c, const double* y1, const double* y2, const PairClassArgs& ca, unsigned pair0, const void** out) {
    auto key = std::make_tuple(len, (int)c, pair0);
    auto it = ctx->split16.find(key);
    if (it != ctx->split16.end()) { *out = it->second; return SSW_OK; }
    void* p = nullptr;
    SSW_ALLOC(&p, base_energy_split_bytes(ca.NP, ca.Kp, pair0));
    const int rc = launch_base_energy_split(ctx->stream, y1, y2, ca.yrows, ca.NP, ca.Kp, pair0, p);
    untimed_work(ctx);
    if (rc != SSW_OK) { (void)hipFree(p); return rc; }
    ctx->split16[key] = p;
    *out = p;
    return SSW_OK;
}

bool valid_method(int m) { return m == SSW_OPTION1 || m == SSW_OPTION2 || m == SSW_OPTION3; }
bool valid_ordering(int o) { return o == SSW_ORDER_ENERGY || o == SSW_ORDER_ENERGY_ORTHOGONAL || o == SSW_ORDER_LEGACY; }
bool valid_precision(int p) { return p == SSW_PRECISION_F32 || p == SSW_PRECISION_F64; }

int check_config(const ssw_config* cfg) {
    if (!cfg) return SSW_ERR_BAD_ARG;
    if (cfg->method == SSW_METHOD_CUSTOM || cfg->ordering == SSW_ORDER_CUSTOM) return SSW_ERR_UNSUPPORTED;
    if (!valid_method(cfg->method) || !valid_ordering(cfg->ordering) || !valid_precision(cfg->precision))
        return SSW_ERR_BAD_ARG;
    return SSW_OK;
}

namespace {
size_t lane_bytes_held(const ssw_ctx* ctx) {
    size_t held = 0;
    for (const auto& ln : ctx->lane) {
        for (const auto& b : ln.plane) held += b.bytes;
        for (const auto& b : ln.operand) held += b.bytes;
        for (const auto& b : ln.compact) held += b.bytes;
        held += ln.idx.bytes + ln.gathered.bytes + ln.prune_u32.bytes;
    }
    return held;
}
}

size_t effective_chunk(const ssw_ctx* ctx, size_t w, size_t h, size_t n_frames) {
    size_t c = ctx->chunk_frames;
    if (c == 0) {
        const size_t px = std::max<size_t>(w * h, 1);
        c = std::max<size_t>(1, ((size_t)1 << 30) / px);
        const size_t per_frame = dct_pair_operand_elems(1, w, h) * sizeof(double);
        if (per_frame) c = std::max<size_t>(1, std::min(c, (size_t)0xFFFFFFFFull / per_frame));
        if (c >= 16) c &= ~(size_t)7;
        c = std::min(c, std::max<size_t>(n_frames, 1));
        size_t free_b = 0, total_b = 0;
        DeviceGuard g(ctx->device);
        if (hipMemGetInfo(&free_b, &total_b) == hipSuccess) {
            const size_t budget = (free_b + lane_bytes_held(ctx) + ctx->plane_pool_bytes) / 2;
            size_t c1 = std::max<size_t>(1, std::min(c, budget / (44 * px)));
            if (ctx->overlap && n_frames > c1) c1 = std::max<size_t>(1, std::min(c1, budget / (2 * 44 * px)));
            c = c1;
        } else {
            (void)hipGetLastError();
        }
    }
    return std::min(c, std::max<size_t>(n_frames, 1));
}

namespace {

bool aligned_planes(const float* a, const float* b) { return ((reinterpret_cast<uintptr_t>(a) | reinterpret_cast<uintptr_t>(b)) & 15) == 0; }
struct PassBuild {
    ssw_ctx* ctx; Xform x; PassPlan p;
    bool first_pass, is_row, inverse, from_rgb;
    size_t n, w, h, len, lines;
    const float* src; float* dst; Epilogue ep;
    int st_pass, st_main, st_prep;
    double px, prep_bytes, out_bpp;
    double gemm_bytes(double xch) const { return px * (8.0 + xch + out_bpp); }
    double flop(PairClass c) const { return pair_class_flop(c, lines, len); }
    PairLayout gemm_layout() const { return is_row ? p.layout : PairLayout(); }
    int gemm(hipStream_t st, int nc, const PairClassDesc* d, double* tmp = nullptr, double* tmp_out = nullptr, const RgbSink* sink = nullptr,
             const PairLayout& lay = PairLayout()) const {
        return launch_dct_pair_gemm_multi_f64(st, is_row, inverse, nc, d, dst, tmp, n, w, h, ep, sink, tmp_out, lay);
    }
    RowInput row_input() const { return from_rgb ? RowInput::rgb(x.rgb_fmt, x.rgb, x.iq_i, x.iq_q) : RowInput::plane(src); }
};

template <class Launch>
int launch_classes(ssw_ctx* ctx, hipStream_t st, bool merge, int nc, const PairClassDesc* d, Launch launch, int st_main = -1,
                   double f_main = 0.0) {
    if (merge) return launch(nc, d);
    for (int c = 0; c + 1 < nc; ++c) SSW_TRY(launch(1, &d[c]));
    if (st_main < 0) return launch(1, &d[nc - 1]);
    StageTimer tm(ctx, st_main, st, f_main);
    return launch(1, &d[nc - 1]);
}

RgbSink rgb_sink(const PassBuild& b, bool* fused_rgb) {
    RgbSink sink;
    if (b.inverse && !b.first_pass && !b.is_row && b.x.rgb_out && b.x.iq_i && b.x.iq_q) {
        sink.iq_i = b.x.iq_i; sink.iq_q = b.x.iq_q; sink.rgb = b.x.rgb_out; sink.u8 = b.x.rgb_out_u8;
        if (fused_rgb) *fused_rgb = true;
    }
    return sink;
}

int class_desc(ssw_ctx* ctx, size_t len, bool inverse, PairClass c, const double* x1, const double* x2, PairClassDesc& d) {
    const PairClassRow& r = pair_class_row(c);
    const void *y1 = nullptr, *y2 = nullptr;
    SSW_TRY(get_basis(ctx, len / r.ydiv, inverse, true, r.y1, &y1));
    if (r.samex) y2 = (const char*)y1 + (len / r.ldiv / r.np_div) * 64;
    else SSW_TRY(get_basis(ctx, len / r.ydiv, inverse, true, r.y2, &y2));
    d = {c, x1, x2, (const double*)y1, (const double*)y2};
    return SSW_OK;
}

struct PairPlanes {
    size_t bytes = 0, p8 = 0, p16 = 0;
    const void* rot = nullptr;
    double *sp = nullptr, *l2 = nullptr;
    size_t l2_plane = 0;
    const double* plane(bool level2, int j) const {
        return level2 ? l2 + (size_t)j * l2_plane : j < 6 ? sp + (size_t)j * p8 : sp + 6 * p8 + (size_t)(j - 6) * p16;
    }
};
int pair_planes(const PassBuild& b, ssw_ctx::Lane& ws, PairPlanes& pp) {
    pp.bytes = dct_pair_operand_elems(b.n, b.w, b.h) * sizeof(double);
    if (!b.p.split) return SSW_OK;
// ... 9 lines not shown
}
int deep_desc(const PassBuild& b, const PairPlanes& pp, bool level2, PairClass c, PairClassDesc& d) {
    const signed char* x = level2 ? pair_class_row(c).l2x : pair_class_row(c).l1x;
    if (x[0] < 0 || !pp.sp) return SSW_ERR_BAD_ARG;
    return class_desc(b, c, pp.plane(level2, x[0]), pp.plane(level2, x[1]), d);
}
int deep_descs(const PassBuild& b, const PairPlanes& pp, bool level2, std::initializer_list<PairClass> cls, PairClassDesc* d) {
    for (PairClass c : cls) SSW_TRY(deep_desc(b, pp, level2, c, *d++));
    return SSW_OK;
}
int deep_rot(const PassBuild& b, bool level2, const void** rot2, const void** rot3) {
    SSW_TRY(get_basis(b.ctx, b.len / 2, false, true, BasisKind::Rot, rot2));
    return level2 ? get_basis(b.ctx, b.len / 4, false, true, BasisKind::Rot, rot3) : SSW_OK;
}

struct OddHalfLaunch { PairClassDesc d[2]; int n = 0; double flop = 0.0; };
int odd_half(const PassBuild& b, const PairPlanes& pp, const double* odd, OddHalfLaunch& o) {
    if (!b.p.split) {
        o.n = 1; o.flop = b.flop(PairClass::OddHalf);
        return class_desc(b, PairClass::OddHalf, odd, odd, o.d[0]);
    }
    o.n = 2; o.flop = b.flop(PairClass::E) + b.flop(PairClass::O);
    return deep_descs(b, pp, false, {PairClass::E, PairClass::O}, o.d);
}
int odd_rotate(const PassBuild& b, const PairPlanes& pp, hipStream_t st, const double* odd) {
    return b.p.split ? launch_dct_pair_rotate(st, odd, (const double*)pp.rot, pp.sp, b.lines, b.len) : SSW_OK;
}
int odd_gemm(const PassBuild& b, const OddHalfLaunch& o, hipStream_t st, double* tmpE, const RgbSink* sink) {
    for (int c = 0; c < o.n; ++c) SSW_TRY(b.gemm(st, 1, &o.d[c], tmpE, nullptr, sink));
    return SSW_OK;
}

int build_dense(const PassBuild& b, Chain& ch) {
    ssw_ctx* ctx = b.ctx;
    const void* b0 = nullptr;
    SSW_TRY(get_basis(ctx, b.len, b.inverse, b.x.precision == SSW_PRECISION_F64, BasisKind::Dense, &b0));
    const double flop = 2.0 * (double)b.lines * (double)b.len * (double)b.len;
    ch.push_back({false, [=](hipStream_t st) -> int {
        StageTimer t(ctx, b.st_pass, st, flop);
        t.traffic(b.px * 8.0);
        if (b.is_row) return launch_dct_rows(st, b.x.precision, b.src, b.dst, b.lines, b.w, b0, b.ep);
        return launch_dct_cols(st, b.x.precision, b.src, b.dst, b.n, b.w, b.h, b0, b.ep);
    }});
    return SSW_OK;
}

int build_pair_l1(const PassBuild& b, ssw_ctx::Lane& ws, Chain& ch) {
    ssw_ctx* ctx = b.ctx;
    PairPlanes pp;
    SSW_TRY(pair_planes(b, ws, pp));
    for (int i = 0; i < 2; ++i) SSW_TRY(grow(ws.operand[i], pp.bytes));
    double *x1 = (double*)ws.operand[0].p, *x2 = (double*)ws.operand[1].p;
    ch.push_back({true, [=](hipStream_t st) -> int {
        StageTimer t(ctx, SSW_STAGE_DCT_PREP, st, b.prep_bytes);
        return launch_dct_pair_prep(st, b.is_row, b.inverse, b.src, b.n, b.w, b.h, x1, x2);
    }});
    const double f_main = b.flop(PairClass::OneLevel);
    PairClassDesc d;
    SSW_TRY(class_desc(b, PairClass::OneLevel, x1, x2, d));
    ch.push_back({false, [=](hipStream_t st) -> int {
        StageTimer t(ctx, b.st_pass, st, f_main);
        t.traffic(b.gemm_bytes(0.0));
        StageTimer tm(ctx, b.st_main, st, f_main);
        return b.gemm(st, 1, &d);
    }});
    return SSW_OK;
}

int build_pair_two(const PassBuild& b, ssw_ctx::Lane& ws, Chain& ch, bool* fused_rgb) {
    ssw_ctx* ctx = b.ctx;
    PairPlanes pp;
    SSW_TRY(pair_planes(b, ws, pp));
    for (int i = 1; i < (b.inverse ? 5 : 4); ++i) SSW_TRY(grow(ws.operand[i], pp.bytes));
    double* x2 = (double*)ws.operand[1].p;
    double* xx1 = (double*)ws.operand[2].p;
    double* xx2 = (double*)ws.operand[3].p;
    double* tmpE = (double*)ws.operand[4].p;
    ch.push_back({true, [=](hipStream_t st) -> int {
        StageTimer t(ctx, b.st_prep, st, b.prep_bytes);
        SSW_TRY(launch_dct_pair_prep4(st, b.is_row, b.inverse, b.row_input(), b.n, b.w, b.h, xx1, xx2, x2));
        return odd_rotate(b, pp, st, x2);
    }});
    OddHalfLaunch odd;
    PairClassDesc even;
    SSW_TRY(odd_half(b, pp, x2, odd));
    SSW_TRY(class_desc(b, PairClass::EvenHalf, xx1, xx2, even));
    const double f_main = odd.flop, f_all = f_main + b.flop(PairClass::EvenHalf);
    const RgbSink sink = rgb_sink(b, fused_rgb);
    ch.push_back({false, [=](hipStream_t st) -> int {
        StageTimer t(ctx, b.st_pass, st, f_all);
        t.traffic(b.gemm_bytes(b.inverse ? 8.0 : 0.0));
        SSW_TRY(b.gemm(st, 1, &even, tmpE));
        StageTimer tm(ctx, b.st_main, st, f_main);
        return odd_gemm(b, odd, st, tmpE, sink.rgb ? &sink : nullptr);
    }});
    return SSW_OK;
}

int build_pair_three(const PassBuild& b, ssw_ctx::Lane& ws, Chain& ch) {
    ssw_ctx* ctx = b.ctx;
    PairPlanes pp;
    SSW_TRY(pair_planes(b, ws, pp));
    for (int i = 0; i < 4; ++i) SSW_TRY(grow(ws.operand[i], pp.bytes));
    double *d1 = (double*)ws.operand[1].p, *d2 = (double*)ws.operand[0].p, *r1 = (double*)ws.operand[2].p, *r2 = (double*)ws.operand[3].p;
    ch.push_back({true, [=](hipStream_t st) -> int {
        StageTimer t(ctx, b.st_prep, st, b.prep_bytes);
        if (!b.is_row) SSW_TRY(launch_dct_pair_prep8_cols(st, b.src, b.n, b.w, b.h, r1, r2, d2, d1));
        else SSW_TRY(launch_dct_pair_prep8_rows(st, b.row_input(), b.n, b.w, b.h, r1, r2, d2, d1));
        return odd_rotate(b, pp, st, d1);
    }});
    OddHalfLaunch odd;
    PairClassDesc r, m;
    SSW_TRY(odd_half(b, pp, d1, odd));
    SSW_TRY(class_desc(b, PairClass::R1R2, r1, r2, r));
    SSW_TRY(class_desc(b, PairClass::OddHalf2, d2, d2, m));
    const double f_main = odd.flop, f_all = f_main + b.flop(PairClass::R1R2) + b.flop(PairClass::OddHalf2);
    ch.push_back({false, [=](hipStream_t st) -> int {
        StageTimer t(ctx, b.st_pass, st, f_all);
        t.traffic(b.gemm_bytes(0.0));
        SSW_TRY(b.gemm(st, 1, &r));
        SSW_TRY(b.gemm(st, 1, &m));
        StageTimer tm(ctx, b.st_main, st, f_main);
        return odd_gemm(b, odd, st, nullptr, nullptr);
    }});
    return SSW_OK;
}


int build_deep(const PassBuild& b, ssw_ctx::Lane& ws, Chain& ch) {
    typedef PairClass C;
    ssw_ctx* ctx = b.ctx;
    PairPlanes pp;
    const void *rot2 = nullptr, *rot3 = nullptr;
    SSW_TRY(pair_planes(b, ws, pp));
    SSW_TRY(deep_rot(b, false, &rot2, &rot3));
    double* sp = pp.sp;
    ch.push_back({true, [=](hipStream_t st) -> int {
        StageTimer t(ctx, b.st_prep, st, b.prep_bytes);
        if (!b.is_row) return launch_dct_pair_prep16_cols(st, b.src, b.n, b.w, b.h, sp, (const double*)pp.rot, (const double*)rot2, nullptr, b.p.prep, b.p.layout);
        return launch_dct_pair_prep16_rows(st, b.row_input(), b.n, b.w, b.h, sp, (const double*)pp.rot, (const double*)rot2, nullptr, false);
    }});
    const double f_main = b.flop(C::O), f_all = f_main + b.flop(C::E) + b.flop(C::R1R2) + b.flop(C::E2) + b.flop(C::O2);
    std::array<PairClassDesc, 5> merged, single;
    SSW_TRY(deep_descs(b, pp, false, {C::R1R2, C::E2, C::O2, C::O, C::E}, merged.data()));
    SSW_TRY(deep_descs(b, pp, false, {C::R1R2, C::E2, C::O2, C::E, C::O}, single.data()));
    ch.push_back({false, [=](hipStream_t st) -> int {
        StageTimer t(ctx, b.st_pass, st, f_all);
        t.traffic(b.gemm_bytes(0.0));
        auto launch = [&](int nc, const PairClassDesc* d) { return b.gemm(st, nc, d, nullptr, nullptr, nullptr, b.gemm_layout()); };
        if (!b.p.merge) return launch_classes(ctx, st, false, 5, single.data(), launch, b.st_main, f_main);
        StageTimer tm(ctx, b.st_main, st, f_all);
        return launch(5, merged.data());
    }});
    return SSW_OK;
}

int build_deep_l2(const PassBuild& b, ssw_ctx::Lane& ws, Chain& ch) {
    ssw_ctx* ctx = b.ctx;
    const bool fused = b.p.strategy == PassStrategy::FusedRows || b.p.strategy == PassStrategy::FusedCols;
    PairPlanes pp;
    const void *rot2 = nullptr, *rot3 = nullptr;
    SSW_TRY(pair_planes(b, ws, pp));
    SSW_TRY(deep_rot(b, true, &rot2, &rot3));
    const size_t n = b.n, w = b.w, h = b.h;
    FuseCols fc;
    const bool bprune = fused && b.x.base_prune != nullptr;
    BasePrune bp = bprune ? *b.x.base_prune : BasePrune();
    double pad = 1.0;
    double bytes = b.gemm_bytes(0.0);
    float* out = b.dst;
    if (fused) {
        const size_t cplane = n * w * dct_pair_split_kpad(h / 2);
        SSW_TRY(grow(ws.operand[0], 16 * cplane * sizeof(double)));
        double* cop = (double*)ws.operand[0].p;
        fc = FuseCols{FUSE_COLS};
        if (!b.is_row) { pp.l2 = cop; pp.l2_plane = cplane; }
        else {
            const void *crot1 = nullptr, *crot2 = nullptr, *crot3 = nullptr;
            SSW_TRY(get_basis(ctx, h, false, true, BasisKind::Rot, &crot1));
            SSW_TRY(get_basis(ctx, h / 2, false, true, BasisKind::Rot, &crot2));
            SSW_TRY(get_basis(ctx, h / 4, false, true, BasisKind::Rot, &crot3));
            const size_t lpad = n * 16 * dct_pair_fused_units(h);
            pp.l2_plane = lpad * dct_pair_split_kpad(b.len / 2);
            pad = (double)lpad / (double)(n * h);
            fc = FuseCols{FUSE_ROWS_COP, cop, (const double*)crot1, (const double*)crot2, (const double*)crot3};
            if (bprune) fc.energy = bp.energy;
            bytes = b.px * 16.0;
            out = nullptr;
        }
    }
    double* sp = pp.sp;
    if (!fused || b.is_row)
        ch.push_back({true, [=](hipStream_t st) -> int {
            StageTimer t(ctx, b.st_prep, st, b.prep_bytes);
            if (!b.is_row) return launch_dct_pair_prep16_cols(st, b.src, n, w, h, sp, (const double*)pp.rot, (const double*)rot2, (const double*)rot3,
                                                              b.p.prep, b.p.layout);
            return launch_dct_pair_prep16_rows(st, b.row_input(), n, w, h, sp, (const double*)pp.rot, (const double*)rot2, (const double*)rot3, true, fused);
        }});
    const double f_main = b.flop(PairClass::O5), f_all = 8.0 * f_main;
    std::array<PairClassDesc, 8> d;
    for (int c = 0; c < 8; ++c) SSW_TRY(deep_desc(b, pp, true, kLevel2Classes[c], d[c]));
    if (bprune && !b.is_row) {
        const double tiles = (double)(w / SSW_BASE_PRUNE_TILE);
        bp.tile_flop = f_all / ((double)n * tiles);
        bp.tile_bytes = bytes / ((double)n * tiles);
        bp.select_bytes = (double)h * SSW_BASE_PRUNE_TILE * 4.0;
        if (bp.decided) *bp.decided = true;
        auto phase = [=](hipStream_t st, int mode) {
            FuseCols f2 = fc;
            f2.tile_mode = mode; f2.need = bp.need;
            return launch_dct_pair_gemm_multi_f64(st, false, false, 8, d.data(), out, nullptr, n, w, h, b.ep, nullptr, nullptr, b.gemm_layout(), &f2);
        };
        ch.push_back({false, [=](hipStream_t st) -> int {
            StageTimer t(ctx, b.st_pass, st, f_all / tiles);
            t.traffic(bytes / tiles);
            return phase(st, 1);
        }});
        ch.push_back({true, [=](hipStream_t st) -> int {
            StageTimer t(ctx, SSW_STAGE_SELECT, st, (double)n * ((double)h * SSW_BASE_PRUNE_TILE + (double)w) * 4.0);
            return launch_base_prune_decide(st, out, bp, n, w, h);
        }});
        if (bp.tail && *bp.tail) {
            const std::function<int(hipStream_t)> tail = *bp.tail;
            ch.push_back({false, [=](hipStream_t st) -> int {
                StageTimer t(ctx, SSW_STAGE_DCT_ROW, st, 0.0);
                return tail(st);
            }});
        }
        ch.push_back({false, [=](hipStream_t st) -> int {
            StageTimer t(ctx, b.st_pass, st, 0.0);
            return phase(st, 2);
        }});
        return SSW_OK;
    }
    if (bprune && bp.tail) *bp.tail = nullptr;
    if (bprune && b.is_row && bp.tail && tuning(TUNE_BASE_ENERGY_LOWP) != 0) {
        std::array<BaseEnergyClass, 8> be;
        bool ok = true;
        unsigned pair0 = 0, np = 0;
        double chunks = 1.0;
        for (int c = 0; c < 8 && ok; ++c) {
            PairClassArgs ca;
            PairInstance inst;
            SSW_TRY(pair_class_args(d[c].cls, true, false, b.len, b.gemm_layout(), false, false, tuning(TUNE_TILE48) != 0, ca, inst));
            const unsigned p0 = ca.bn32 == 2 ? 48u : 64u;
            ok = ca.tiles_n >= 2 && ca.Kp <= 256 && ca.gsh <= 16 && ca.bn32 != 1 && ca.np1 == 0xFFFFFFFFu && ca.p2lo == 0 && ca.pm <= 1 &&
                 (c == 0 || (p0 == pair0 && ca.NP == np));
            if (!ok) break;
            pair0 = p0; np = ca.NP;
            const void* y16 = nullptr;
            SSW_TRY(get_split16(ctx, b.len, d[c].cls, d[c].y1, d[c].y2, ca, pair0, &y16));
            be[c].x1 = d[c].x1; be[c].x2 = d[c].x2; be[c].y16 = y16;
            be[c].NP = ca.NP; be[c].Kp = ca.Kp; be[c].pair0 = pair0; be[c].pm = ca.pm; be[c].c1 = ca.c1; be[c].c2 = ca.c2; be[c].gsh = ca.gsh; be[c].e2off = ca.e2off;
            chunks = (double)(((ca.NP - pair0 + 15) / 16 + 10) / 11);
        }
        if (ok) {
            const size_t lpf = 16 * dct_pair_fused_units(h);
            const double head = (double)pair0 / (double)np;
            const double bound_bytes = 8.0 * 2.0 * chunks * (double)(n * lpf) * (double)be[0].Kp * 8.0;
            unsigned long long* tail_stats = bp.stats ? bp.stats + 8 : nullptr;
            const double tail_flop = 4.0 * (double)lpf * (double)(b.len / 16), tail_bytes = 16.0 * (double)h;
            ch.push_back({false, [=](hipStream_t st) -> int {
                SSW_HIP_CHECK(hipMemsetAsync(bp.energy, 0, n * w * sizeof(float), st));
                untimed_work(ctx);
                {
                    StageTimer tp(ctx, SSW_STAGE_DCT_PREP, st, bound_bytes);
                    SSW_TRY(launch_base_energy_bound(st, 8, be.data(), n, w, h, lpf, b.ep.base, bp.energy));
                }
                FuseCols fh = fc;
                fh.row_part = 1;
                StageTimer t(ctx, b.st_pass, st, f_all * pad * head);
                t.traffic(b.px * 8.0 * (1.0 + head));
                auto launch = [&](int nc, const PairClassDesc* dd) {
                    return launch_dct_pair_gemm_multi_f64(st, true, false, nc, dd, out, nullptr, n, w, h, b.ep, nullptr, nullptr, b.gemm_layout(), &fh);
                };
                return launch_classes(ctx, st, b.p.merge, 8, d.data(), launch);
            }});
            const PairLayout lay = b.gemm_layout();
            const Epilogue ep = b.ep;
            const bool merge = b.p.merge;
            *bp.tail = [=](hipStream_t st) -> int {
                FuseCols ft = fc;
                ft.row_part = 2; ft.energy = nullptr; ft.need = bp.need;
                ft.tail = tail_stats; ft.tail_flop = tail_flop; ft.tail_bytes = tail_bytes;
                auto launch = [&](int nc, const PairClassDesc* dd) {
                    return launch_dct_pair_gemm_multi_f64(st, true, false, nc, dd, out, nullptr, n, w, h, ep, nullptr, nullptr, lay, &ft);
                };
                return launch_classes(ctx, st, merge, 8, d.data(), launch);
            };
            return SSW_OK;
        }
    }
    ch.push_back({false, [=](hipStream_t st) -> int {
        if (bprune) {
            SSW_HIP_CHECK(hipMemsetAsync(bp.energy, 0, n * w * sizeof(float), st));
            untimed_work(ctx);
        }
        StageTimer t(ctx, b.st_pass, st, f_all * pad, b.p.merge ? b.st_main : -1);
        t.traffic(bytes);
        auto launch = [&](int nc, const PairClassDesc* dd) {
            return launch_dct_pair_gemm_multi_f64(st, b.is_row, false, nc, dd, out, nullptr, n, w, h, b.ep, nullptr, nullptr, b.gemm_layout(),
                                                  fused ? &fc : nullptr);
        };
        return launch_classes(ctx, st, b.p.merge, 8, d.data(), launch, b.st_main, f_main * pad);
    }});
    return SSW_OK;
}

int build_semi_deep(const PassBuild& b, ssw_ctx::Lane& ws, Chain& ch, bool* fused_rgb) {
    typedef PairClass C;
    ssw_ctx* ctx = b.ctx;
    const bool inv = b.inverse;
    PairPlanes pp;
    SSW_TRY(pair_planes(b, ws, pp));
    if (inv) for (int i : {1, 4}) SSW_TRY(grow(ws.operand[i], pp.bytes));
    double* T2 = inv ? (double*)ws.operand[1].p : nullptr;
    double* TE = inv ? (double*)ws.operand[4].p : nullptr;
    double* sp = pp.sp;
    const double* rot = (const double*)pp.rot;
    ch.push_back({true, [=](hipStream_t st) -> int {
        StageTimer t(ctx, b.st_prep, st, b.prep_bytes);
        if (inv) return launch_dct_pair_prep16_inv_cols(st, b.src, b.n, b.w, b.h, sp, rot, rot, nullptr, b.p.prep, b.p.layout);
        return launch_dct_pair_prep16_cols(st, b.src, b.n, b.w, b.h, sp, rot, rot, nullptr, b.p.prep, b.p.layout);
    }});
    const RgbSink sink = rgb_sink(b, fused_rgb);
    PairClassDesc r1, sd, eo[2];
    SSW_TRY(deep_desc(b, pp, false, C::R1R2, r1));
    SSW_TRY(deep_desc(b, pp, false, C::OddHalf2, sd));
    SSW_TRY(deep_descs(b, pp, false, {C::E, C::O}, eo));
    const double f_sd = b.flop(C::OddHalf2);
    const double f_main = b.flop(C::E), f_all = f_main + b.flop(C::O) + b.flop(C::R1R2) + f_sd;
    ch.push_back({false, [=](hipStream_t st) -> int {
        StageTimer t(ctx, b.st_pass, st, f_all);
        t.traffic(b.gemm_bytes(inv ? 12.0 : 0.0));
        if (inv) {
            SSW_TRY(b.gemm(st, 1, &r1, T2));
            SSW_TRY(b.gemm(st, 1, &sd, T2, TE));
            return launch_classes(ctx, st, b.p.merge, 2, eo, [&](int nc, const PairClassDesc* d) { return b.gemm(st, nc, d, TE, nullptr, sink.rgb ? &sink : nullptr); });
        }
        if (b.p.merge) {
            SSW_TRY(b.gemm(st, 1, &sd));
            const PairClassDesc d[3] = {r1, eo[1], eo[0]};
            StageTimer tm(ctx, b.st_main, st, f_all - f_sd);
            return b.gemm(st, 3, d);
        }
        SSW_TRY(b.gemm(st, 1, &r1));
        SSW_TRY(b.gemm(st, 1, &sd));
        SSW_TRY(b.gemm(st, 1, &eo[1]));
        StageTimer tm(ctx, b.st_main, st, f_main);
        return b.gemm(st, 1, &eo[0]);
    }});
    return SSW_OK;
}

int build_deep_inv(const PassBuild& b, ssw_ctx::Lane& ws, Chain& ch, bool* fused_rgb) {
    typedef PairClass C;
    ssw_ctx* ctx = b.ctx;
    const bool l2 = b.p.strategy == PassStrategy::DeepInvL2;
    const size_t len = b.len, lines = b.lines;
    PairPlanes pp;
    const void *rot2 = nullptr, *rot3 = nullptr;
    SSW_TRY(pair_planes(b, ws, pp));
    SSW_TRY(deep_rot(b, l2, &rot2, &rot3));
    SSW_TRY(grow(ws.operand[1], std::max<size_t>(pp.bytes, lines * (len / 4) * sizeof(double))));
    SSW_TRY(grow(ws.operand[4], std::max<size_t>(pp.bytes, lines * (len / 2) * sizeof(double))));
    double* A1 = nullptr;
    if (l2) {
        SSW_TRY(grow(ws.operand[2], std::max<size_t>(pp.bytes, lines * (len / 8) * sizeof(double))));
        A1 = (double*)ws.operand[2].p;
    }
    double* T2 = (double*)ws.operand[1].p;
    double* TE = (double*)ws.operand[4].p;
    double* sp = pp.sp;
    const RgbSink sink = rgb_sink(b, fused_rgb);
    ch.push_back({true, [=](hipStream_t st) -> int {
        StageTimer t(ctx, b.st_prep, st, b.prep_bytes);
        if (!b.is_row) return launch_dct_pair_prep16_inv_cols(st, b.src, b.n, b.w, b.h, sp, (const double*)pp.rot, (const double*)rot2, (const double*)rot3,
                                                              b.p.prep, b.p.layout);
        return launch_dct_pair_prep16_inv_rows(st, b.src, b.n, b.w, b.h, sp, (const double*)pp.rot, (const double*)rot2, (const double*)rot3, b.p.prep);
    }});
    PairClassDesc da{}, dt, d1[2], d0[4];
    if (l2) SSW_TRY(deep_desc(b, pp, true, C::R1A, da));
    SSW_TRY(deep_desc(b, pp, l2, l2 ? C::R2A : C::R1R2, dt));
    SSW_TRY(deep_descs(b, pp, l2, {C::E2, C::O2}, d1));
    if (l2) SSW_TRY(deep_descs(b, pp, true, {C::EE, C::EO, C::O5, C::O3}, d0));
    else SSW_TRY(deep_descs(b, pp, false, {C::E, C::O}, d0));
    const double f_all = l2 ? 8.0 * b.flop(C::O5) : b.flop(C::E) + b.flop(C::O) + b.flop(C::R1R2) + b.flop(C::E2) + b.flop(C::O2);
    const std::array<PairClassDesc, 2> s1{d1[0], d1[1]};
    const std::array<PairClassDesc, 4> s0{d0[0], d0[1], d0[2], d0[3]};
    ch.push_back({false, [=](hipStream_t st) -> int {
        StageTimer t(ctx, b.st_pass, st, f_all);
        t.traffic(b.gemm_bytes(l2 ? 14.0 : 12.0));
        const PairLayout lay = b.gemm_layout();
        if (l2) SSW_TRY(b.gemm(st, 1, &da, A1));
        SSW_TRY(l2 ? b.gemm(st, 1, &dt, A1, T2, nullptr, lay) : b.gemm(st, 1, &dt, T2));
        SSW_TRY(launch_classes(ctx, st, b.p.merge, 2, s1.data(), [&](int nc, const PairClassDesc* d) { return b.gemm(st, nc, d, T2, TE, nullptr, lay); }));
        return launch_classes(ctx, st, b.p.merge, l2 ? 4 : 2, s0.data(),
                              [&](int nc, const PairClassDesc* d) { return b.gemm(st, nc, d, TE, nullptr, sink.rgb ? &sink : nullptr, lay); });
    }});
    return SSW_OK;
}

int build_pass(ssw_ctx* ctx, ssw_ctx::Lane& ws, const Xform& x, bool first_pass, bool is_row, const float* src, float* dst,
               Epilogue ep, Chain& ch, bool* fused_rgb = nullptr) {
    const PlanInput in{x.type, x.precision, x.n, x.w, x.h, x.full_h, x.natural_order, aligned_planes(src, dst), plan_settings(ctx)};
    PassBuild b{ctx, x, plan_pass(in, first_pass, is_row), first_pass, is_row, x.type == SSW_DCT3, x.rgb && first_pass, x.n, x.w, x.h,
                is_row ? x.w : x.h, is_row ? x.n * x.h : x.n * x.w, src, dst, ep};
    if (b.from_rgb && !(is_row && b.p.levels >= 2)) return SSW_ERR_BAD_ARG;
    b.st_pass = is_row ? SSW_STAGE_DCT_ROW : SSW_STAGE_DCT_COL;
    b.st_main = is_row ? SSW_STAGE_DCT_ROW_MAIN : SSW_STAGE_DCT_COL_MAIN;
    b.st_prep = b.from_rgb ? SSW_STAGE_RGB_TO_YIQ : SSW_STAGE_DCT_PREP;
    b.px = (double)b.n * (double)b.w * (double)b.h;
    b.prep_bytes = b.from_rgb ? b.px * (3.0 * (double)pix_bytes(x.rgb_fmt) + (x.iq_i ? 8.0 : 0.0) + 8.0) : b.px * (4.0 + 8.0);
    const bool sink_pass = b.inverse && !first_pass && !is_row && x.rgb_out && x.iq_i && x.iq_q;
    b.out_bpp = sink_pass ? 8.0 + 3.0 * (x.rgb_out_u8 ? 1.0 : 4.0) : 4.0;
    const size_t first = ch.size();
    typedef PassStrategy S;
    const S s = b.p.strategy;
    SSW_TRY(s == S::Dense                   ? build_dense(b, ch)
            : s == S::PairL1                ? build_pair_l1(b, ws, ch)
            : s == S::PairTwo               ? build_pair_two(b, ws, ch, fused_rgb)
            : s == S::PairThree             ? build_pair_three(b, ws, ch)
            : s == S::Deep                  ? build_deep(b, ws, ch)
            : s == S::SemiDeep || s == S::SemiDeepInv ? build_semi_deep(b, ws, ch, fused_rgb)
            : s == S::DeepInv || s == S::DeepInvL2    ? build_deep_inv(b, ws, ch, fused_rgb)
                                                      : build_deep_l2(b, ws, ch));
    for (size_t i = first; i < ch.size(); ++i) {
        if (!ch[i].hbm && is_row) ch[i].tag = 1;
        if (ch[i].hbm && is_row && first_pass && x.type != SSW_DCT3 && x.rgb) ch[i].tag = 2;
    }
    return SSW_OK;
}

}

int build_transform(ssw_ctx* ctx, ssw_ctx::Lane& ws, const Xform& x, Chain& ch, bool* fused_rgb) {
    const bool f64 = (x.precision == SSW_PRECISION_F64);
    const size_t n = x.n, w = x.w, h = x.h;
    if (n == 0) return SSW_OK;
    const size_t max_frames = plan_frame_limit(plan_settings(ctx), f64, w, h);
    if (n > max_frames) {
        for (size_t f0 = 0; f0 < n; f0 += max_frames) {
            Xform s = x;
            s.n = std::min(max_frames, n - f0);
            s.data = x.data + f0 * w * h;
            s.tmp = x.tmp + f0 * w * h;
            if (x.rgb) s.rgb = static_cast<const char*>(x.rgb) + f0 * w * h * 3 * pix_bytes(x.rgb_fmt);
            if (x.iq_i) s.iq_i = x.iq_i + f0 * w * h;
            if (x.iq_q) s.iq_q = x.iq_q + f0 * w * h;
            if (x.rgb_out) s.rgb_out = static_cast<char*>(x.rgb_out) + f0 * w * h * 3 * (x.rgb_out_u8 ? 1 : sizeof(float));
            SSW_TRY(build_transform(ctx, ws, s, ch, fused_rgb));
        }
        return SSW_OK;
    }
    const bool rows_first = (w >= h);
    Epilogue plain{1.f, 1.f};
    auto ortho = [&](size_t len) {
        Epilogue e{std::sqrt(1.0f / (4.0f * (float)len)), std::sqrt(1.0f / (2.0f * (float)len))};
// ... 307 lines not shown
        if (!(frag ? want_frag : want_natural)) continue;
        PruneGatherJobs jobs;
        jobs.n = 0;
        for (unsigned i = 0; i < t.plan.n_classes; ++i) {
            jobs.j[jobs.n++] = t.gather(i, frag, false);
            if (t.c[i].s.split) jobs.j[jobs.n++] = t.gather(i, frag, true);
        }
        SSW_TRY(launch_prune_gather_bases(st, jobs));
    }
    return SSW_OK;
}

int make_call_prune_tables(ssw_ctx* ctx, const PruneSetup& ps, size_t w, size_t k, const uint32_t* idx, uint32_t* info) {
    PruneTables t;
    SSW_TRY(lay_out_prune_tables(ctx, nullptr, ps, w, info, t));
    untimed_work(ctx);
    return enqueue_prune_tables(ctx->stream, t, idx, 1, k, true, plan_is_level2(ps.rows));
}

struct PrunedChunk {
    ssw_ctx* ctx;
    RowInput in;
    size_t n, w, h, k, lines;
    const uint32_t* idx;
    bool make_tables;
    double *sp, *o[4];
    float* t_compact;
    PruneTables t;
    size_t cap() const { return t.plan.cap_total; }
    double px() const { return (double)n * (double)w * (double)h; }
    double rgb_bytes() const { return px() * 3.0 * (double)pix_bytes(pix_fmt(in.kind)); }
};

void pruned_rows_fused(const PrunedChunk& q, const std::array<DerivedFusedClass, 9>& fca, Chain& ch) {
    ssw_ctx* ctx = q.ctx;
    if (q.make_tables)
        ch.push_back({true, [=](hipStream_t st) -> int {
            untimed_work(ctx);
            return enqueue_prune_tables(st, q.t, q.idx, q.n, q.k, false, true);
        }});
    const double in_bytes = q.rgb_bytes();
    ch.push_back({false, [=](hipStream_t st) -> int {
        StageTimer t(ctx, SSW_STAGE_RGB_TO_YIQ, st, in_bytes + (double)q.lines * (double)q.cap() * 4.0);
        return launch_dct_pair_derived_fused(st, q.in, q.lines, q.w, q.t.rot[0], q.t.rot[1], q.t.rot[2], q.t.plan.n_classes, fca.data(),
                                             q.t_compact, (unsigned)q.cap());
    }});
}

void pruned_rows_gathered(const PrunedChunk& q, Chain& ch) {
    ssw_ctx* ctx = q.ctx;
    const bool deep = plan_is_deep(q.t.rows), level2 = plan_is_level2(q.t.rows);
    const int levels = q.t.rows.levels;
    const unsigned ncl = q.t.plan.n_classes;
    const double prep_bytes = q.rgb_bytes() + q.px() * 8.0;
    double flop = 0.0;
    for (unsigned c = 0; c < ncl; ++c) flop += (q.t.c[c].s.split ? 4.0 : 2.0) * (double)q.lines * q.t.plan.c[c].cap * (double)q.t.c[c].s.ktrue;
    ch.push_back({true, [=](hipStream_t st) -> int {
        if (q.make_tables) {
            SSW_TRY(enqueue_prune_tables(st, q.t, q.idx, q.n, q.k, false, false));
            untimed_work(ctx);
        }
        StageTimer t(ctx, SSW_STAGE_RGB_TO_YIQ, st, prep_bytes);
        if (deep) return launch_dct_pair_prep16_rows(st, q.in, q.n, q.w, q.h, q.sp, q.t.rot[0], q.t.rot[1], q.t.rot[2], level2);
        if (levels == 3) SSW_TRY(launch_dct_pair_prep8_rows(st, q.in, q.n, q.w, q.h, q.o[2], q.o[3], q.o[0], q.o[1]));
        else SSW_TRY(launch_dct_pair_prep4(st, true, false, q.in, q.n, q.w, q.h, q.o[2], q.o[3], q.o[1]));
        return q.sp ? launch_dct_pair_rotate(st, q.o[1], q.t.rot[0], q.sp, q.lines, q.w) : SSW_OK;
    }});
    ch.back().tag = 2;
    ch.push_back({false, [=](hipStream_t st) -> int {
        if (q.make_tables) {
            SSW_TRY(enqueue_prune_tables(st, q.t, nullptr, 0, 0, true, false));
            untimed_work(ctx);
        }
        StageTimer t(ctx, SSW_STAGE_DCT_ROW, st, flop);
        t.traffic(q.px() * 8.0 + (double)q.lines * (double)q.cap() * 4.0);
        if (plan_merge(q.lines)) {
            PairSubsetClass sc[9];
            for (unsigned c = 0; c < ncl; ++c) sc[c] = q.t.subset(c);
            return launch_dct_pair_gemm_rows_subset_merged_f64(st, sc, ncl, q.t_compact, (unsigned)q.cap(), q.lines);
        }
        for (unsigned c = 0; c < ncl; ++c) {
            const PairSubsetClass s = q.t.subset(c);
            if (s.x2) SSW_TRY(launch_dct_pair_gemm_rows_subset_split_f64(st, s.x1, s.x2, s.y1, s.y2, s.cap, s.Kp, q.t_compact, (unsigned)q.cap(), s.off, q.lines));
            else SSW_TRY(launch_dct_pair_gemm_rows_subset_f64(st, s.x1, s.y1, s.cap, s.Kp, q.t_compact, (unsigned)q.cap(), s.off, q.lines));
        }
        return SSW_OK;
    }});
}

int pruned_cols(ssw_ctx* ctx, ssw_ctx::Lane& ws, size_t n, size_t cap, size_t h, Chain& ch) {
    float *t_compact = (float*)ws.compact[0].p, *compact = (float*)ws.compact[1].p;
    Xform xc{SSW_DCT2, SSW_PRECISION_F64, n, cap, h, compact, t_compact};
    xc.natural_order = true;
    return build_pass(ctx, ws, xc, false, false, t_compact, compact, Epilogue{1.f, 1.f}, ch);
}

int build_pruned_derived(ssw_ctx* ctx, ssw_ctx::Lane& ws, const void* rgb, PixFmt fmt, size_t n, size_t w, size_t h, size_t k,
                         const uint32_t* idx, const PruneSetup& ps, uint32_t* info, bool call_tables, Chain& ch, const uint32_t** pos) {
    const size_t cap = ps.plan.cap_total, lines = n * h;
    const bool deep = plan_is_deep(ps.rows), level2 = plan_is_level2(ps.rows);
    if (!deep) for (int b = 0; b < 4; ++b) SSW_TRY(grow(ws.operand[b], dct_pair_operand_elems(n, w, h) * sizeof(double)));
    for (int b = 0; b < 2; ++b) SSW_TRY(grow(ws.compact[b], n * h * cap * sizeof(float)));
    if (ps.rows.split) SSW_TRY(grow(ws.operand[5], split_scratch_elems(n, w, h) * sizeof(double)));
    PrunedChunk q{ctx, RowInput::rgb(fmt, rgb), n, w, h, k, lines, idx, !call_tables, ps.rows.split ? (double*)ws.operand[5].p : nullptr,
                  {(double*)ws.operand[0].p, (double*)ws.operand[1].p, (double*)ws.operand[2].p, (double*)ws.operand[3].p}, (float*)ws.compact[0].p};
    SSW_TRY(lay_out_prune_tables(ctx, call_tables ? nullptr : &ws, ps, w, info, q.t));
    *pos = q.t.pos;
    PairPlanes pp;
    pp.sp = pp.l2 = q.sp;
    pp.p8 = lines * dct_pair_split_kpad(w);
    pp.p16 = pp.l2_plane = lines * dct_pair_split_kpad(w / 2);
    for (unsigned c = 0; c < ps.plan.n_classes; ++c) {
        const PruneClassSrc& s = ps.src[c];
        q.t.c[c].x = s.lane_buf >= 0 ? q.o[s.lane_buf] : pp.plane(level2, s.p1);
        q.t.c[c].x2 = s.split ? pp.plane(level2, s.p2) : nullptr;
    }
    std::array<DerivedFusedClass, 9> fca{};
    if (level2) for (unsigned c = 0; c < 9; ++c) fca[c] = q.t.fused(c < ps.plan.n_classes ? c : 0);
    if (level2 && plan_derived_fused(ps.rows, lines) && dct_pair_derived_fused_fits(ps.plan.n_classes, fca.data())) pruned_rows_fused(q, fca, ch);
    else pruned_rows_gathered(q, ch);
    return pruned_cols(ctx, ws, n, cap, h, ch);
}

typedef std::function<int(size_t, ssw_ctx::Lane&, Chain&, bool)> PrunedChunkBuilder;
int run_pruned_pipeline(ssw_ctx* ctx, size_t n_chunks, const PruneSetup& ps, bool info_per_chunk, const PrunedChunkBuilder& build_chunk) {
    SSW_TRY(run_pipeline(ctx, n_chunks, [&](size_t ci, ssw_ctx::Lane& ws, Chain& ch) { return build_chunk(ci, ws, ch, ps.on); }));
    if (!ps.on) return SSW_OK;
    std::vector<uint32_t> info((info_per_chunk ? n_chunks : 1) * SSW_PRUNE_INFO);
    SSW_HIP_CHECK(hipMemcpyAsync(info.data(), ctx->overflow.p, info.size() * sizeof(uint32_t), hipMemcpyDeviceToHost, ctx->stream));
    SSW_HIP_CHECK(hipStreamSynchronize(ctx->stream));
    for (size_t ci = 0; ci < n_chunks; ++ci) {
        const uint32_t* block = info.data() + (info_per_chunk ? ci : 0) * SSW_PRUNE_INFO;
        ctx->pruned_chunks++;
        if (info_per_chunk || ci == 0)
            for (unsigned q = 0; q < ps.plan.n_classes; ++q) ctx->pruned_columns += block[1 + q];
        if (block[0] == 0) continue;
        ctx->redone_chunks++;
        Chain ch;
        SSW_TRY(build_chunk(ci, ctx->lane[0], ch, false));
        SSW_TRY(run_serial(ch, ctx->stream));
    }
    return SSW_OK;
}

bool base_prune_shape_ok(const ssw_ctx* ctx, const ssw_config& c, size_t n, size_t w, size_t h, const void* rgb, PixFmt fmt, const float* y, const float* tmp) {
    const bool f64 = c.precision == SSW_PRECISION_F64;
    if (!f64 || w % SSW_BASE_PRUNE_TILE != 0 || w / SSW_BASE_PRUNE_TILE < 2 || w < h || !(base_prune_gain(w, h, c.ordering) > 0.0f)) return false;
    if (!can_fuse_rgb(ctx, f64, w, h, y, tmp, rgb, fmt)) return false;
    const PlanInput in{SSW_DCT2, c.precision, n, w, h, 0, false, true, plan_settings(ctx)};
    return n <= plan_frame_limit(plan_settings(ctx), f64, w, h) && plan_pass(in, true, true).strategy == PassStrategy::FusedRows &&
           plan_pass(in, false, false).strategy == PassStrategy::FusedCols;
}
int base_prune_workspace(ssw_ctx::Lane& ws, size_t frames, size_t w, BasePrune& bp) {
    const size_t e_bytes = frames * w * sizeof(float);
    SSW_TRY(grow(ws.base_prune, e_bytes + frames * (w / SSW_BASE_PRUNE_TILE) * sizeof(unsigned)));
    bp.energy = (float*)ws.base_prune.p;
    bp.need = (unsigned*)((char*)ws.base_prune.p + e_bytes);
    return SSW_OK;
}

void push_extract_stage(Chain& ch, ssw_ctx* ctx, const ssw_config& c, const float* yb, const float* derived, const uint32_t* pos, size_t cap,
                        size_t n, size_t w, size_t h, const uint32_t* idx, size_t k, float* ext, const float* marks, float* sims) {
    ch.push_back({true, [=](hipStream_t st) -> int {
        if (k > 0) {
            StageTimer t(ctx, SSW_STAGE_EXTRACT, st);
            if (pos) SSW_TRY(launch_extract_pruned(st, yb, derived, n, w, h, cap, pos, idx, k, c.method, c.alpha, ext));
            else SSW_TRY(launch_extract(st, yb, derived, n, w * h, idx, k, c.method, c.alpha, ext));
        }
        if (marks) {
            StageTimer t(ctx, SSW_STAGE_SIMILARITY, st);
            SSW_TRY(launch_similarity(st, ext, marks, n, k, sims));
        }
        return SSW_OK;
    }});
}

}

int batch_embed_impl(ssw_ctx* ctx, const ssw_config* cfg, const void* dev_rgb, PixFmt fmt_in, size_t n_frames, size_t w,
                     size_t h, const float* dev_marks, size_t k, void* dev_rgb_out, bool u8_out, float* dev_coef_out,
                     uint32_t* dev_indices_out) {
    if (!ctx || !dev_rgb || !dev_marks || !dev_rgb_out) return SSW_ERR_BAD_ARG;
    SSW_TRY(check_config(cfg));
    if (w == 0 || h == 0) return SSW_ERR_BAD_DIMS;
    const size_t plane = w * h;
    const size_t k_eff = std::min(k, plane - 1);
    CtxGuard g(ctx);
    const size_t chunk = effective_chunk(ctx, w, h, n_frames);
    const size_t n_chunks = (n_frames + chunk - 1) / chunk;
    const ssw_config c = *cfg;
    const size_t in_px = 3 * pix_bytes(fmt_in), out_px = u8_out ? 3 : 3 * sizeof(float);
    auto build = [&](size_t ci, ssw_ctx::Lane& ws, Chain& ch) -> int {
        const size_t f0 = ci * chunk, n = std::min(chunk, n_frames - f0);
        for (int p = 0; p < 4; ++p) SSW_TRY(grow(ws.plane[p], chunk * plane * sizeof(float)));
        SSW_TRY(grow(ws.idx, chunk * std::max<size_t>(k_eff, 1) * sizeof(uint32_t)));
        float* y = (float*)ws.plane[0].p;
        float* pi = (float*)ws.plane[1].p;
        float* pq = (float*)ws.plane[2].p;
        float* tmp = (float*)ws.plane[3].p;
        const char* rgb = static_cast<const char*>(dev_rgb) + f0 * plane * in_px;
        char* out = static_cast<char*>(dev_rgb_out) + f0 * plane * out_px;
        uint32_t* idx = dev_indices_out ? dev_indices_out + f0 * k_eff : (uint32_t*)ws.idx.p;
        float* coef_out = dev_coef_out ? dev_coef_out + f0 * plane : nullptr;
        const float* marks = dev_marks + f0 * k;
        SelectWorkspace* sel = &ws.sel;
        SSW_TRY(build_forward_from_rgb(ctx, ws, c.precision, rgb, fmt_in, n, w, h, y, pi, pq, tmp, ch));
        ch.push_back({true, [=](hipStream_t st) -> int {
            if (coef_out) { SSW_HIP_CHECK(hipMemcpyAsync(coef_out, y, n * plane * sizeof(float), hipMemcpyDeviceToDevice, st)); untimed_work(ctx); }
            if (k_eff == 0) return SSW_OK;
            SSW_TRY(topk(ctx, st, *sel, y, n, w, h, c.ordering, k_eff, idx));
            StageTimer t(ctx, SSW_STAGE_EMBED, st);
            return launch_embed(st, y, n, plane, idx, k_eff, marks, nullptr, nullptr, 1, k_eff, k, c.method, c.alpha);
        }});
        Xform inv{SSW_DCT3, c.precision, n, w, h, y, tmp};
        inv.iq_i = pi; inv.iq_q = pq; inv.rgb_out = out; inv.rgb_out_u8 = u8_out;
        bool fused_rgb = false;
        SSW_TRY(build_transform(ctx, ws, inv, ch, &fused_rgb));
        if (fused_rgb) return SSW_OK;
        const double out_bytes = (double)n * plane * (12.0 + (u8_out ? 3.0 : 12.0));
        ch.push_back({true, [=](hipStream_t st) -> int {
            StageTimer t(ctx, SSW_STAGE_YIQ_TO_RGB, st, out_bytes);
            if (u8_out) return launch_yiq_to_rgb8(st, y, pi, pq, n * plane, reinterpret_cast<uint8_t*>(out));
            return launch_yiq_to_rgb(st, y, pi, pq, n * plane, reinterpret_cast<float*>(out));
        }});
        return SSW_OK;
    };
    return run_pipeline(ctx, n_chunks, build);
}

int batch_extract_impl(ssw_ctx* ctx, const ssw_config* cfg, const void* dev_base_rgb, const void* dev_derived_rgb, PixFmt fmt,
                       size_t n_frames, size_t w, size_t h, size_t k, float* dev_extracted, const float* dev_marks,
                       float* dev_sims) {
    if (!ctx || !dev_base_rgb || !dev_derived_rgb || !dev_extracted) return SSW_ERR_BAD_ARG;
    if ((dev_marks == nullptr) != (dev_sims == nullptr)) return SSW_ERR_BAD_ARG;
    SSW_TRY(check_config(cfg));
    if (w == 0 || h == 0) return SSW_ERR_BAD_DIMS;
    const size_t plane = w * h;
    if (k >= plane) return SSW_ERR_K_TOO_LARGE;
    if (n_frames == 0) return SSW_OK;
    CtxGuard g(ctx);
    const size_t chunk = effective_chunk(ctx, w, h, n_frames);
    const size_t n_chunks = (n_frames + chunk - 1) / chunk;
    const ssw_config c = *cfg;
    const bool f64 = c.precision == SSW_PRECISION_F64;
    const size_t px_bytes = 3 * pix_bytes(fmt);
    for (int l = 0; l < (pipeline_uses_two_lanes(ctx, n_chunks) ? 2 : 1); ++l)
        for (int p : {0, 2}) SSW_TRY(grow(ctx->lane[l].plane[p], chunk * plane * sizeof(float)));
    const float *y0 = (const float*)ctx->lane[0].plane[0].p, *tmp0 = (const float*)ctx->lane[0].plane[2].p;
    const PruneSetup ps = stream_capturing(ctx) ? PruneSetup() : make_prune_setup(ctx, f64, std::min(chunk, n_frames), w, h, k, y0, tmp0, dev_derived_rgb, fmt);
    if (ps.on) SSW_TRY(grow(ctx->overflow, n_chunks * SSW_PRUNE_INFO * sizeof(uint32_t)));
    uint32_t* overflow = (uint32_t*)ctx->overflow.p;
    bool base_prune = ctx->prune && tuning(TUNE_BASE_PRUNE) != 0 && k > 0 && k <= select_max_k();
    for (size_t f0 = 0; base_prune && f0 < n_frames; f0 += chunk)
        base_prune = base_prune_shape_ok(ctx, c, std::min(chunk, n_frames - f0), w, h, dev_base_rgb, fmt, y0, tmp0);
    if (base_prune && !ctx->base_prune_stats.p) {
        SSW_TRY(grow(ctx->base_prune_stats, SSW_BASE_PRUNE_STATS * sizeof(unsigned long long)));
        SSW_HIP_CHECK(hipMemsetAsync(ctx->base_prune_stats.p, 0, SSW_BASE_PRUNE_STATS * sizeof(unsigned long long), ctx->stream));
        untimed_work(ctx);
    }

    auto build_chunk = [&](size_t ci, ssw_ctx::Lane& ws, Chain& ch, bool pruned) -> int {
        const size_t f0 = ci * chunk, n = std::min(chunk, n_frames - f0);
        for (int p : {0, 2}) SSW_TRY(grow(ws.plane[p], chunk * plane * sizeof(float)));
        SSW_TRY(grow(ws.idx, chunk * std::max<size_t>(k, 1) * sizeof(uint32_t)));
        float* yb = (float*)ws.plane[0].p;
        float* tmp = (float*)ws.plane[2].p;
        uint32_t* idx = (uint32_t*)ws.idx.p;
        const char* brgb = static_cast<const char*>(dev_base_rgb) + f0 * plane * px_bytes;
        const char* drgb = static_cast<const char*>(dev_derived_rgb) + f0 * plane * px_bytes;
        SelectWorkspace* sel = &ws.sel;
        BasePrune bp;
        bool decided = false;
        std::function<int(hipStream_t)> tail;
        if (base_prune) {
            bp.decided = &decided;
            bp.tail = &tail;
            SSW_TRY(base_prune_workspace(ws, chunk, w, bp));
            bp.stats = (unsigned long long*)ctx->base_prune_stats.p;
            bp.work = (double*)(bp.stats + 4);
            bp.k = k; bp.ordering = c.ordering;
        }
        SSW_TRY(build_forward_from_rgb(ctx, ws, c.precision, brgb, fmt, n, w, h, yb, nullptr, nullptr, tmp, ch, base_prune ? &bp : nullptr));
        const unsigned* mask = decided ? bp.need : nullptr;
        if (k > 0)
            ch.push_back({true, [=](hipStream_t st) -> int { return topk(ctx, st, *sel, yb, n, w, h, c.ordering, k, idx, mask); }});
        const float* derived = nullptr;
        const uint32_t* pos = nullptr;
        if (pruned) {
            SSW_TRY(build_pruned_derived(ctx, ws, drgb, fmt, n, w, h, k, idx, ps, overflow + ci * SSW_PRUNE_INFO, false, ch, &pos));
            derived = (const float*)ws.compact[1].p;
        } else {
            SSW_TRY(grow(ws.plane[1], chunk * plane * sizeof(float)));
            SSW_TRY(build_forward_from_rgb(ctx, ws, c.precision, drgb, fmt, n, w, h, (float*)ws.plane[1].p, nullptr, nullptr, tmp, ch));
            derived = (const float*)ws.plane[1].p;
        }
        push_extract_stage(ch, ctx, c, yb, derived, pos, ps.plan.cap_total, n, w, h, idx, k, dev_extracted + f0 * k,
                           dev_marks ? dev_marks + f0 * k : nullptr, dev_sims ? dev_sims + f0 : nullptr);
        return SSW_OK;
    };
    return run_pruned_pipeline(ctx, n_chunks, ps, true, build_chunk);
}

int base_prune_bound_impl(ssw_ctx* ctx, const ssw_config* cfg, const float* dev_rgb, size_t n_frames, size_t w, size_t h, size_t k,
                          float* dev_bound) {
    const ssw_config c = *cfg;
    if (w == 0 || h == 0) return SSW_ERR_BAD_DIMS;
    if (n_frames == 0) return SSW_OK;
    const size_t plane = w * h;
    ssw_ctx::Lane& ws = ctx->lane[0];
    for (int p : {0, 2}) SSW_TRY(grow(ws.plane[p], n_frames * plane * sizeof(float)));
    if (k == 0 || k >= plane || !base_prune_shape_ok(ctx, c, n_frames, w, h, dev_rgb, PixFmt::F32, (const float*)ws.plane[0].p, (const float*)ws.plane[2].p))
        return SSW_ERR_UNSUPPORTED;
    BasePrune bp;
    std::function<int(hipStream_t)> tail;
    SSW_TRY(base_prune_workspace(ws, n_frames, w, bp));
    bp.k = k; bp.ordering = c.ordering;
    bp.tail = &tail;
    Chain ch;
    SSW_TRY(build_forward_from_rgb(ctx, ws, c.precision, dev_rgb, PixFmt::F32, n_frames, w, h, (float*)ws.plane[0].p, nullptr, nullptr,
                                   (float*)ws.plane[2].p, ch, &bp));
    SSW_TRY(run_serial(ch, ctx->stream));
    untimed_work(ctx);
    return launch_base_prune_bound(ctx->stream, bp.energy, n_frames, w, h, c.ordering, dev_bound);
}

int trace_base(ssw_ctx* ctx, const ssw_config& c, const void* dev_base_rgb, PixFmt fmt, size_t w, size_t h, size_t k, const float** y,
               const uint32_t** idx) {
    const size_t plane = w * h;
    ssw_ctx::Lane& ws = ctx->lane[0];
    SSW_TRY(grow(ctx->trace[0], plane * sizeof(float)));
    SSW_TRY(grow(ctx->trace[1], std::max<size_t>(k, 1) * sizeof(uint32_t)));
    SSW_TRY(grow(ws.plane[2], plane * sizeof(float)));
    float* yb = (float*)ctx->trace[0].p;
    uint32_t* ib = (uint32_t*)ctx->trace[1].p;
    Chain ch;
    SSW_TRY(build_forward_from_rgb(ctx, ws, c.precision, dev_base_rgb, fmt, 1, w, h, yb, nullptr, nullptr, (float*)ws.plane[2].p, ch));
    SSW_TRY(run_serial(ch, ctx->stream));
    if (k > 0) SSW_TRY(topk(ctx, ctx->stream, ws.sel, yb, 1, w, h, c.ordering, k, ib));
    *y = yb;
    *idx = ib;
    return SSW_OK;
}

int trace_extract(ssw_ctx* ctx, const ssw_config& c, const float* yb, const uint32_t* idx, const void* dev_suspect_rgb, PixFmt fmt,
                  size_t n_frames, size_t w, size_t h, size_t k, float* dev_extracted) {
    if (n_frames == 0) return SSW_OK;
    const size_t plane = w * h;
    const size_t chunk = effective_chunk(ctx, w, h, n_frames);
    const size_t n_chunks = (n_frames + chunk - 1) / chunk;
    const size_t px_bytes = 3 * pix_bytes(fmt);
    const PruneSetup ps = stream_capturing(ctx) ? PruneSetup()
                          : make_prune_setup(ctx, c.precision == SSW_PRECISION_F64, std::min(chunk, n_frames), w, h, k, yb, yb, dev_suspect_rgb, fmt);
    if (ps.on) SSW_TRY(grow(ctx->overflow, SSW_PRUNE_INFO * sizeof(uint32_t)));
    uint32_t* info = (uint32_t*)ctx->overflow.p;
    if (ps.on) SSW_TRY(make_call_prune_tables(ctx, ps, w, k, idx, info));
    auto build_chunk = [&](size_t ci, ssw_ctx::Lane& ws, Chain& ch, bool pruned) -> int {
        const size_t f0 = ci * chunk, n = std::min(chunk, n_frames - f0);
        const char* srgb = static_cast<const char*>(dev_suspect_rgb) + f0 * plane * px_bytes;
        float* ext = dev_extracted + f0 * k;
        const uint32_t* pos = nullptr;
        if (pruned) SSW_TRY(build_pruned_derived(ctx, ws, srgb, fmt, n, w, h, k, idx, ps, info, true, ch, &pos));
        else {
            for (int p : {1, 2}) SSW_TRY(grow(ws.plane[p], chunk * plane * sizeof(float)));
// ... 42 lines not shown
```

### spread_spectrum_watermarking_amd/csrc/tuning.hip

```cpp
#include <atomic>
#include <cstdlib>
#include <cstring>
#include <mutex>

#include "ssw_internal.hpp"

namespace ssw {
namespace {

struct Entry {
    const char* name;
    const char* env;
    long long dflt;
    std::atomic<long long> value{0};
    std::atomic<int> state{0};
    Entry(const char* n, const char* e, long long d) : name(n), env(e), dflt(d) {}
};

Entry g_tune[TUNE_COUNT] = {
    {"efold_min", "SSW_EFOLD_MIN", 1280},
    {"efold_inv_min", "SSW_EFOLD_INV_MIN", 1280},
    {"efold_cols_min", "SSW_EFOLD_COLS_MIN", 720},
    {"class_tile", "SSW_CLASS_TILE", 1},
    {"deep_min_rows", "SSW_DEEP_MIN_ROWS", 256},
    {"deep_min_cols", "SSW_DEEP_MIN_COLS", 256},
    {"prep_staged", "SSW_PREP_STAGED", 1},
    {"merge_max_lines", "SSW_MERGE_MAX_LINES", 8192},
    {"bn32", "SSW_BN32", -1},
    {"band_split", "SSW_BAND_SPLIT", 1},
    {"fuse_cols", "SSW_FUSE_COLS", 1},
    {"upload_bands", "SSW_UPLOAD_BANDS", 3},
    {"speculate_k", "SSW_SPECULATE_K", 1},
    {"prep_light", "SSW_PREP_LIGHT", 1},
    {"lane_stagger", "SSW_LANE_STAGGER", 1},
    {"derived_fused", "SSW_DERIVED_FUSED", 1},
    {"tile48", "SSW_TILE48", 1},
    {"base_prune", "SSW_BASE_PRUNE", 1},
    {"base_energy_lowp", "SSW_BASE_ENERGY_LOWP", 1},
};

std::mutex g_tune_lock;

}

long long tuning(int which) {
    Entry& e = g_tune[which];
    if (e.state.load(std::memory_order_acquire) == 0) {
        std::lock_guard<std::mutex> lk(g_tune_lock);
        if (e.state.load(std::memory_order_relaxed) == 0) {
            const char* s = std::getenv(e.env);
            long long v = s ? std::atoll(s) : e.dflt;
            if (which == TUNE_BAND_SPLIT && std::getenv("SSW_NO_SPLIT")) v = 0;
            e.value.store(v, std::memory_order_relaxed);
            e.state.store(1, std::memory_order_release);
        }
    }
    return e.value.load(std::memory_order_relaxed);
}

}

extern "C" {

int ssw_tuning_set(const char* name, long long value) {
    if (!name) return SSW_ERR_BAD_ARG;
    for (int i = 0; i < ssw::TUNE_COUNT; ++i)
        if (std::strcmp(ssw::g_tune[i].name, name) == 0) {
            std::lock_guard<std::mutex> lk(ssw::g_tune_lock);
            ssw::g_tune[i].value.store(value, std::memory_order_relaxed);
            ssw::g_tune[i].state.store(2, std::memory_order_release);
            return SSW_OK;
        }
    return SSW_ERR_BAD_ARG;
}

int ssw_tuning_get(const char* name, long long* value) {
    if (!name || !value) return SSW_ERR_BAD_ARG;
    for (int i = 0; i < ssw::TUNE_COUNT; ++i)
        if (std::strcmp(ssw::g_tune[i].name, name) == 0) { *value = ssw::tuning(i); return SSW_OK; }
    return SSW_ERR_BAD_ARG;
}

int ssw_tuning_reset(const char* name) {
    for (int i = 0; i < ssw::TUNE_COUNT; ++i)
        if (!name || std::strcmp(ssw::g_tune[i].name, name) == 0) {
            std::lock_guard<std::mutex> lk(ssw::g_tune_lock);
            ssw::g_tune[i].state.store(0, std::memory_order_release);
            if (name) return SSW_OK;
        }
    return name ? SSW_ERR_BAD_ARG : SSW_OK;
}

}
```

Measured before the change: 17780.

## Compact pruned column tiles into a job list and mask top-k in writer path

The prune decision kernel now writes the needed tile indices into a compacted job list with an atomic counter. The second-phase fused column DCT launches a grid capped near twice the CU count and loops persistently over only those jobs, instead of launching every tile and returning early. A separate writer-path mask runs the prune decision after full column transforms so top-k selection can skip tiles that cannot hold the winners. The cost is extra atomics, an in-kernel barrier loop, and more device-to-host stat reads, with a risk of load imbalance when the job count is small.

```diff
diff --git a/spread_spectrum_watermarking_amd/csrc/base_prune.hip b/spread_spectrum_watermarking_amd/csrc/base_prune.hip
--- a/spread_spectrum_watermarking_amd/csrc/base_prune.hip
+++ b/spread_spectrum_watermarking_amd/csrc/base_prune.hip
@@ -27,7 +27,8 @@
                                                                        unsigned W, unsigned H, BpKey kp, unsigned k,
                                                                        unsigned* __restrict__ need, unsigned long long* __restrict__ stats,
                                                                        double* __restrict__ work, double tile_flop, double tile_bytes,
-                                                                       double select_bytes) {
+                                                                       double select_bytes, unsigned* __restrict__ jobs,
+                                                                       unsigned* __restrict__ njobs, double* __restrict__ select_work) {
     __shared__ unsigned hist[BP_BINS];
     __shared__ unsigned part[BP_THREADS / 64];
     __shared__ float t_sh;
@@ -83,18 +84,30 @@
         if (!(T > 1e-30f) || !(bound < T)) { nd[x / SSW_BASE_PRUNE_TILE] = 1u; any_sh = 1u; }
     }
     __syncthreads();
-    if (tid == 0 && stats) {
+    if (tid == 0 && jobs) {
+        unsigned mine = 0;
+        for (unsigned t = 1; t < tiles; ++t) mine += nd[t];
+        if (mine) {
+            unsigned at = atomicAdd(njobs, mine);
+            for (unsigned t = 1; t < tiles; ++t)
+                if (nd[t]) jobs[at++] = f * tiles + t;
+        }
+    }
+    if (tid == 0 && (stats || select_work)) {
         unsigned computed = 0;
         for (unsigned t = 0; t < tiles; ++t) computed += nd[t];
-        if (work) {
-            if (computed > 1) {
-                atomicAdd(&work[0], (computed - 1) * tile_flop); atomicAdd(&work[1], (computed - 1) * tile_bytes);
-                atomicAdd(&work[2], (computed - 1) * select_bytes);
+        if (stats) {
+            if (work) {
+                if (computed > 1) {
+                    atomicAdd(&work[0], (computed - 1) * tile_flop); atomicAdd(&work[1], (computed - 1) * tile_bytes);
+                    atomicAdd(&work[2], (computed - 1) * select_bytes);
+                }
             }
+            atomicAdd(&stats[0], (unsigned long long)tiles);
+            atomicAdd(&stats[1], (unsigned long long)computed);
+            if (any_sh) atomicAdd(&stats[2], 1ull);
         }
-        atomicAdd(&stats[0], (unsigned long long)tiles);
-        atomicAdd(&stats[1], (unsigned long long)computed);
-        if (any_sh) atomicAdd(&stats[2], 1ull);
+        if (select_work && computed > 1) atomicAdd(select_work, (computed - 1) * select_bytes);
     }
 }
 
@@ -138,11 +151,12 @@
 int launch_base_prune_decide(hipStream_t st, const float* coef, const BasePrune& bp, size_t n_frames, size_t w, size_t h) {
     if (n_frames == 0) return SSW_OK;
     if (!coef || !bp.energy || !bp.need || (reinterpret_cast<uintptr_t>(coef) & 15) != 0 || w % SSW_BASE_PRUNE_TILE != 0 || w > 0xFFFFFFull || h > 0xFFFFFFull || n_frames > 0x7FFFFFFFull ||
-        bp.k == 0 || bp.k > 0xFFFFFFFFull) return SSW_ERR_BAD_ARG;
+        bp.k == 0 || bp.k > 0xFFFFFFFFull || (bp.njobs && !bp.jobs) || n_frames * (w / SSW_BASE_PRUNE_TILE) > 0xFFFFFFFFull) return SSW_ERR_BAD_ARG;
     const BpKey kp = make_key(w, h, bp.ordering);
     if (!(kp.gain > 0.0f)) return SSW_ERR_BAD_ARG;
     base_prune_decide_kernel<<<(unsigned)n_frames, BP_THREADS, 0, st>>>(coef, bp.energy, (unsigned)w, (unsigned)h, kp, (unsigned)bp.k, bp.need,
-                                                                       bp.stats, bp.work, bp.tile_flop, bp.tile_bytes, bp.select_bytes);
+                                                                       bp.stats, bp.work, bp.tile_flop, bp.tile_bytes, bp.select_bytes,
+                                                                       bp.njobs ? bp.jobs : nullptr, bp.njobs, bp.select_work);
     SSW_HIP_CHECK(hipGetLastError());
     return SSW_OK;
 }
diff --git a/spread_spectrum_watermarking_amd/csrc/dct_pair_f64.hip b/spread_spectrum_watermarking_amd/csrc/dct_pair_f64.hip
--- a/spread_spectrum_watermarking_amd/csrc/dct_pair_f64.hip
+++ b/spread_spectrum_watermarking_amd/csrc/dct_pair_f64.hip
@@ -1,5 +1,6 @@
 #include "dct_pair_common.hpp"
 
+#include <algorithm>
 #include <cstdlib>
 #include <type_traits>
 
@@ -95,8 +96,12 @@
         const bool bn32 = force >= 0 ? force != 0 : 0.92 * balance((unsigned long long)tiles_m * tn32) > balance((unsigned long long)tiles_m * tiles_n);
         if (bn32) { ml.c[0].tiles_n = tiles_n = tn32; ml.c[0].bn32 = 1; }
     }
-    const unsigned long long nblk = (unsigned long long)tiles_m * tiles_n;
+    unsigned long long nblk = (unsigned long long)tiles_m * tiles_n;
     if (nblk > 0x7FFFFFFFull) return SSW_ERR_BAD_DIMS;
+    if (fuse_cols && fuse->tile_mode == 3) {
+        if (!fuse->jobs || !fuse->njobs || fuse->job_grid == 0) return SSW_ERR_BAD_ARG;
+        nblk = std::min<unsigned long long>(nblk, ((unsigned long long)fuse->job_grid + 7u) / 8u * 8u);
+    }
     ml.n_classes = (unsigned)n_classes; ml.L = L; ml.tiles_m = tiles_m; ml.tiles_n_total = tiles_n;
     PairOut po{out, tmp, (unsigned)w, (unsigned)h, (unsigned)(inverse ? leff0 : len), 0, 1, 2};
     po.tmp_out = tmp_out;
@@ -117,8 +122,10 @@
     po.col_energy = energy ? fuse->energy : nullptr;
     ml.need = nullptr; ml.need_mode = 0; ml.need_tpf = 1;
     if (fuse_cols && fuse->tile_mode) {
-        if (inst.epi != EPI_FWD || inst.samex || small || (fuse->tile_mode == 2 && !fuse->need)) return SSW_ERR_BAD_ARG;
+        if (inst.epi != EPI_FWD || inst.samex || small || (fuse->tile_mode == 2 && !fuse->need) || fuse->tile_mode < 1 || fuse->tile_mode > 3)
+            return SSW_ERR_BAD_ARG;
         ml.need = fuse->need; ml.need_mode = (unsigned)fuse->tile_mode; ml.need_tpf = (unsigned)(w / 128);
+        ml.jobs = fuse->jobs; ml.njobs = fuse->njobs;
     }
     if (row_part == 2) {
         if (energy || po.ft != 128) return SSW_ERR_BAD_ARG;
diff --git a/spread_spectrum_watermarking_amd/csrc/dct_pair_f64_kernel.hpp b/spread_spectrum_watermarking_amd/csrc/dct_pair_f64_kernel.hpp
--- a/spread_spectrum_watermarking_amd/csrc/dct_pair_f64_kernel.hpp
+++ b/spread_spectrum_watermarking_amd/csrc/dct_pair_f64_kernel.hpp
@@ -28,6 +28,8 @@
     PairOut po;
     const unsigned* need = nullptr;
     unsigned need_mode = 0, need_tpf = 1;
+    const unsigned* jobs = nullptr;
+    const unsigned* njobs = nullptr;
     unsigned long long* tail = nullptr;
     double tail_flop = 0.0, tail_bytes = 0.0;
 };
@@ -54,11 +56,23 @@
     if (threadIdx.x == 0 && g_tile_trace) kslot = atomicAdd(&g_tile_trace_n, 1u);
 #endif
     SSW_TT(0);
+    constexpr bool JOBS = COLS && EPI == EPI_FWD && BM == 128 && SUB >= 10;
+    unsigned vb = blockIdx.x, vgrid = gridDim.x, tiles_m = ml.tiles_m;
+    if constexpr (JOBS) {
+        if (ml.need_mode == 3) {
+            const unsigned nj = *ml.njobs;
+            tiles_m = nj < ml.tiles_m ? nj : ml.tiles_m;
+            vgrid = tiles_m * ml.tiles_n_total;
+            if (vb >= vgrid) return;
+        }
+    }
+    for (;;) {
     unsigned tm, tn, cls = 0;
-    tile_of_block(blockIdx.x, gridDim.x, ml.tiles_m, ml.tiles_n_total, tm, tn);
+    tile_of_block(vb, vgrid, tiles_m, ml.tiles_n_total, tm, tn);
     while (cls + 1 < ml.n_classes && tn >= ml.c[cls].tiles_n) { tn -= ml.c[cls].tiles_n; ++cls; }
-    if constexpr (COLS && EPI == EPI_FWD && BM == 128 && SUB >= 10) {
+    if constexpr (JOBS) {
         if (ml.need_mode == 1) tm *= ml.need_tpf;
+        else if (ml.need_mode == 3) { const unsigned j = ml.jobs[tm]; tm = j < ml.tiles_m ? j : 0u; }
         else if (tm % ml.need_tpf == 0 || ml.need[tm] == 0) return;
     }
     if constexpr (!COLS && EPI == EPI_FWD_COLOP && SUB == 5) {
@@ -962,6 +976,14 @@
     else if (po.bn32 != 2 && (NP - p0 <= 32 || po.bn32)) run(std::integral_constant<int, BM / 64>{}, J2{});
     else if (j3)                       run(std::integral_constant<int, BM / 64>{}, J3{});
     else                               run(std::integral_constant<int, BM / 32>{}, J2{});
+    if constexpr (!JOBS) break;
+    else {
+        if (ml.need_mode != 3) break;
+        vb += gridDim.x;
+        if (vb >= vgrid) break;
+        asm volatile("s_waitcnt vmcnt(0) lgkmcnt(0)\n\ts_barrier" ::: "memory");
+    }
+    }
 #endif
 }
 
diff --git a/spread_spectrum_watermarking_amd/csrc/ssw_internal.hpp b/spread_spectrum_watermarking_amd/csrc/ssw_internal.hpp
--- a/spread_spectrum_watermarking_amd/csrc/ssw_internal.hpp
+++ b/spread_spectrum_watermarking_amd/csrc/ssw_internal.hpp
@@ -90,6 +90,9 @@
     float* energy = nullptr;
     const unsigned* need = nullptr;
     int tile_mode = 0;
+    const unsigned* jobs = nullptr;
+    const unsigned* njobs = nullptr;
+    unsigned job_grid = 0;
     int row_part = 0;
     unsigned long long* tail = nullptr;
     double tail_flop = 0.0, tail_bytes = 0.0;
@@ -111,7 +114,7 @@
                                                 unsigned out_stride, size_t lines);
 size_t dct_pair_split_kpad(size_t len);
 enum { TUNE_EFOLD_MIN, TUNE_EFOLD_INV_MIN, TUNE_EFOLD_COLS_MIN, TUNE_CLASS_TILE, TUNE_DEEP_MIN_ROWS, TUNE_DEEP_MIN_COLS, TUNE_PREP_STAGED,
-       TUNE_MERGE_MAX_LINES, TUNE_BN32, TUNE_BAND_SPLIT, TUNE_FUSE_COLS, TUNE_UPLOAD_BANDS, TUNE_SPECULATE_K, TUNE_PREP_LIGHT, TUNE_LANE_STAGGER, TUNE_DERIVED_FUSED, TUNE_TILE48, TUNE_BASE_PRUNE, TUNE_BASE_ENERGY_LOWP, TUNE_COUNT };
+       TUNE_MERGE_MAX_LINES, TUNE_BN32, TUNE_BAND_SPLIT, TUNE_FUSE_COLS, TUNE_UPLOAD_BANDS, TUNE_SPECULATE_K, TUNE_PREP_LIGHT, TUNE_LANE_STAGGER, TUNE_DERIVED_FUSED, TUNE_TILE48, TUNE_BASE_PRUNE, TUNE_BASE_ENERGY_LOWP, TUNE_PHASE2_JOBS, TUNE_WRITER_MASK, TUNE_COUNT };
 long long tuning(int which);
 int launch_prep16_cols_l2(hipStream_t st, const float* in, size_t n_frames, size_t w, size_t h, double* base,
                           const double* rot1, const double* rot2, const double* rot3, bool class_major, bool in_l2, unsigned K16);
@@ -173,14 +176,20 @@
 
 constexpr unsigned SSW_BASE_PRUNE_TILE = 128;
 constexpr unsigned SSW_BASE_PRUNE_STATS = 16;
+constexpr unsigned SSW_BASE_PRUNE_WRITER_SELECT = 12;
+constexpr size_t SSW_BASE_PRUNE_HEAD = 256;
 struct BasePrune {
     float* energy = nullptr;
     unsigned* need = nullptr;
+    unsigned* njobs = nullptr;
+    unsigned* jobs = nullptr;
     unsigned long long* stats = nullptr;
     size_t k = 0;
     int ordering = 0;
     double* work = nullptr;
     double tile_flop = 0.0, tile_bytes = 0.0, select_bytes = 0.0;
+    bool full_cols = false;
+    double* select_work = nullptr;
     bool* decided = nullptr;
     std::function<int(hipStream_t)>* tail = nullptr;
 };
@@ -270,6 +279,7 @@
     hipStream_t stream = nullptr;
     hipStream_t own_stream = nullptr;
     size_t chunk_frames = 0;
+    int cu_count = 256;
 
     std::map<std::tuple<size_t, bool, bool, ssw::BasisKind>, void*> basis;
     std::map<std::tuple<size_t, int, unsigned>, void*> split16;
@@ -304,7 +314,7 @@
     uint64_t pruned_chunks = 0, redone_chunks = 0;
     uint64_t pruned_columns = 0;
     Buf base_prune_stats;
-    double base_prune_billed[5] = {0.0, 0.0, 0.0, 0.0, 0.0};
+    double base_prune_billed[6] = {0.0, 0.0, 0.0, 0.0, 0.0, 0.0};
     hipStream_t copy_stream = nullptr;
     struct FrameStage {
         Buf buf;
diff --git a/spread_spectrum_watermarking_amd/csrc/ssw_lib.hip b/spread_spectrum_watermarking_amd/csrc/ssw_lib.hip
--- a/spread_spectrum_watermarking_amd/csrc/ssw_lib.hip
+++ b/spread_spectrum_watermarking_amd/csrc/ssw_lib.hip
@@ -278,7 +278,10 @@
     ssw_ctx* ctx = new (std::nothrow) ssw_ctx();
     if (!ctx) return SSW_ERR_OUT_OF_MEMORY;
     ctx->device = device_id;
-    hipError_t e = hipStreamCreateWithFlags(&ctx->own_stream, hipStreamNonBlocking);
+    int cus = 0;
+    if (hipDeviceGetAttribute(&cus, hipDeviceAttributeMultiprocessorCount, device_id) == hipSuccess && cus > 0) ctx->cu_count = cus;
+    else (void)hipGetLastError();
+    hipError_t e =hipStreamCreateWithFlags(&ctx->own_stream, hipStreamNonBlocking);
     if (e != hipSuccess) { delete ctx; set_last_error(hipGetErrorString(e)); return SSW_ERR_HIP; }
     ctx->stream = ctx->own_stream;
     e = hipStreamCreateWithFlags(&ctx->aux_stream, hipStreamNonBlocking);
diff --git a/spread_spectrum_watermarking_amd/csrc/ssw_pipeline.hip b/spread_spectrum_watermarking_amd/csrc/ssw_pipeline.hip
--- a/spread_spectrum_watermarking_amd/csrc/ssw_pipeline.hip
+++ b/spread_spectrum_watermarking_amd/csrc/ssw_pipeline.hip
@@ -166,6 +166,13 @@
             ctx->stage_bytes[SSW_STAGE_DCT_ROW] += tw[1] - ctx->base_prune_billed[4];
         }
         for (int i = 0; i < 2; ++i) ctx->base_prune_billed[3 + i] = tw[i];
+        double ws = 0.0;
+        SSW_HIP_CHECK(hipMemcpy(&ws, (const char*)ctx->base_prune_stats.p + SSW_BASE_PRUNE_WRITER_SELECT * sizeof(unsigned long long), sizeof(ws), hipMemcpyDeviceToHost));
+        if (ctx->timing) {
+            ctx->stage_work[SSW_STAGE_SELECT] += ws - ctx->base_prune_billed[5];
+            ctx->stage_bytes[SSW_STAGE_SELECT] += ws - ctx->base_prune_billed[5];
+        }
+        ctx->base_prune_billed[5] = ws;
     }
     return SSW_OK;
 }
@@ -481,6 +488,13 @@
         StageTimer tm(ctx, b.st_main, st, f_all);
         return launch(5, merged.data());
     }});
+    return SSW_OK;
+}
+
+int base_prune_zero(hipStream_t st, const BasePrune& bp, size_t n, size_t w) {
+    const bool head = bp.njobs != nullptr;
+    if (head && (char*)bp.njobs + SSW_BASE_PRUNE_HEAD != (char*)bp.energy) return SSW_ERR_BAD_ARG;
+    SSW_HIP_CHECK(hipMemsetAsync(head ? (void*)bp.njobs : (void*)bp.energy, 0, n * w * sizeof(float) + (head ? SSW_BASE_PRUNE_HEAD : 0), st));
     return SSW_OK;
 }
 
@@ -529,15 +543,19 @@
     const double f_main = b.flop(PairClass::O5), f_all = 8.0 * f_main;
     std::array<PairClassDesc, 8> d;
     for (int c = 0; c < 8; ++c) SSW_TRY(deep_desc(b, pp, true, kLevel2Classes[c], d[c]));
-    if (bprune && !b.is_row) {
+    if (bprune && !b.is_row && !bp.full_cols) {
         const double tiles = (double)(w / SSW_BASE_PRUNE_TILE);
         bp.tile_flop = f_all / ((double)n * tiles);
         bp.tile_bytes = bytes / ((double)n * tiles);
         bp.select_bytes = (double)h * SSW_BASE_PRUNE_TILE * 4.0;
         if (bp.decided) *bp.decided = true;
+        const long long jobs_sw = tuning(TUNE_PHASE2_JOBS);
+        if (jobs_sw <= 0 || !bp.jobs) bp.njobs = nullptr;
+        const unsigned job_grid = jobs_sw > 1 ? (unsigned)std::min<long long>(jobs_sw, 1 << 20) : 2u * (unsigned)ctx->cu_count;
         auto phase = [=](hipStream_t st, int mode) {
             FuseCols f2 = fc;
             f2.tile_mode = mode; f2.need = bp.need;
+            f2.jobs = bp.jobs; f2.njobs = bp.njobs; f2.job_grid = job_grid;
             return launch_dct_pair_gemm_multi_f64(st, false, false, 8, d.data(), out, nullptr, n, w, h, b.ep, nullptr, nullptr, b.gemm_layout(), &f2);
         };
         ch.push_back({false, [=](hipStream_t st) -> int {
@@ -558,7 +576,7 @@
         }
         ch.push_back({false, [=](hipStream_t st) -> int {
             StageTimer t(ctx, b.st_pass, st, 0.0);
-            return phase(st, 2);
+            return phase(st, bp.njobs ? 3 : 2);
         }});
         return SSW_OK;
     }
@@ -590,7 +608,7 @@
             unsigned long long* tail_stats = bp.stats ? bp.stats + 8 : nullptr;
             const double tail_flop = 4.0 * (double)lpf * (double)(b.len / 16), tail_bytes = 16.0 * (double)h;
             ch.push_back({false, [=](hipStream_t st) -> int {
-                SSW_HIP_CHECK(hipMemsetAsync(bp.energy, 0, n * w * sizeof(float), st));
+                SSW_TRY(base_prune_zero(st, bp, n, w));
                 untimed_work(ctx);
                 {
                     StageTimer tp(ctx, SSW_STAGE_DCT_PREP, st, bound_bytes);
@@ -621,8 +639,8 @@
         }
     }
     ch.push_back({false, [=](hipStream_t st) -> int {
-        if (bprune) {
-            SSW_HIP_CHECK(hipMemsetAsync(bp.energy, 0, n * w * sizeof(float), st));
+        if (bprune && b.is_row) {
+            SSW_TRY(base_prune_zero(st, bp, n, w));
             untimed_work(ctx);
         }
         StageTimer t(ctx, b.st_pass, st, f_all * pad, b.p.merge ? b.st_main : -1);
@@ -633,6 +651,16 @@
         };
         return launch_classes(ctx, st, b.p.merge, 8, d.data(), launch, b.st_main, f_main * pad);
     }});
+    if (bprune && !b.is_row && bp.full_cols) {
+        bp.njobs = nullptr;
+        bp.tile_flop = bp.tile_bytes = 0.0;
+        bp.select_bytes = (double)h * SSW_BASE_PRUNE_TILE * 4.0;
+        if (bp.decided) *bp.decided = true;
+        ch.push_back({true, [=](hipStream_t st) -> int {
+            StageTimer t(ctx, SSW_STAGE_SELECT, st, (double)n * ((double)h * SSW_BASE_PRUNE_TILE + (double)w) * 4.0);
+            return launch_base_prune_decide(st, out, bp, n, w, h);
+        }});
+    }
     return SSW_OK;
 }
 
@@ -1246,10 +1274,13 @@
            plan_pass(in, false, false).strategy == PassStrategy::FusedCols;
 }
 int base_prune_workspace(ssw_ctx::Lane& ws, size_t frames, size_t w, BasePrune& bp) {
-    const size_t e_bytes = frames * w * sizeof(float);
-    SSW_TRY(grow(ws.base_prune, e_bytes + frames * (w / SSW_BASE_PRUNE_TILE) * sizeof(unsigned)));
-    bp.energy = (float*)ws.base_prune.p;
-    bp.need = (unsigned*)((char*)ws.base_prune.p + e_bytes);
+    const size_t e_bytes = frames * w * sizeof(float), t_bytes = frames * (w / SSW_BASE_PRUNE_TILE) * sizeof(unsigned);
+    SSW_TRY(grow(ws.base_prune, SSW_BASE_PRUNE_HEAD + e_bytes + 2 * t_bytes));
+    char* p = (char*)ws.base_prune.p;
+    bp.njobs = (unsigned*)p;
+    bp.energy = (float*)(p + SSW_BASE_PRUNE_HEAD);
+    bp.need = (unsigned*)(p + SSW_BASE_PRUNE_HEAD + e_bytes);
+    bp.jobs = (unsigned*)(p + SSW_BASE_PRUNE_HEAD + e_bytes + t_bytes);
     return SSW_OK;
 }
 
@@ -1284,6 +1315,16 @@
     const size_t n_chunks = (n_frames + chunk - 1) / chunk;
     const ssw_config c = *cfg;
     const size_t in_px = 3 * pix_bytes(fmt_in), out_px = u8_out ? 3 : 3 * sizeof(float);
+    for (int p : {0, 3}) SSW_TRY(grow(ctx->lane[0].plane[p], chunk * plane * sizeof(float)));
+    const float *y0 = (const float*)ctx->lane[0].plane[0].p, *tmp0 = (const float*)ctx->lane[0].plane[3].p;
+    bool mask_on = tuning(TUNE_WRITER_MASK) != 0 && k_eff > 0 && k_eff <= select_max_k();
+    for (size_t f0 = 0; mask_on && f0 < n_frames; f0 += chunk)
+        mask_on = base_prune_shape_ok(ctx, *cfg, std::min(chunk, n_frames - f0), w, h, dev_rgb, fmt_in, y0, tmp0);
+    if (mask_on && !ctx->base_prune_stats.p) {
+        SSW_TRY(grow(ctx->base_prune_stats, SSW_BASE_PRUNE_STATS * sizeof(unsigned long long)));
+        SSW_HIP_CHECK(hipMemsetAsync(ctx->base_prune_stats.p, 0, SSW_BASE_PRUNE_STATS * sizeof(unsigned long long), ctx->stream));
+        untimed_work(ctx);
+    }
     auto build = [&](size_t ci, ssw_ctx::Lane& ws, Chain& ch) -> int {
         const size_t f0 = ci * chunk, n = std::min(chunk, n_frames - f0);
         for (int p = 0; p < 4; ++p) SSW_TRY(grow(ws.plane[p], chunk * plane * sizeof(float)));
@@ -1298,11 +1339,21 @@
         float* coef_out = dev_coef_out ? dev_coef_out + f0 * plane : nullptr;
         const float* marks = dev_marks + f0 * k;
         SelectWorkspace* sel = &ws.sel;
-        SSW_TRY(build_forward_from_rgb(ctx, ws, c.precision, rgb, fmt_in, n, w, h, y, pi, pq, tmp, ch));
+        BasePrune bp;
+        bool decided = false;
+        if (mask_on) {
+            SSW_TRY(base_prune_workspace(ws, chunk, w, bp));
+            bp.full_cols = true;
+            bp.decided = &decided;
+            bp.select_work = (double*)ctx->base_prune_stats.p + SSW_BASE_PRUNE_WRITER_SELECT;
+            bp.k = k_eff; bp.ordering = c.ordering;
+        }
+        SSW_TRY(build_forward_from_rgb(ctx, ws, c.precision, rgb, fmt_in, n, w, h, y, pi, pq, tmp, ch, mask_on ? &bp : nullptr));
+        const unsigned* mask = decided ? bp.need : nullptr;
         ch.push_back({true, [=](hipStream_t st) -> int {
             if (coef_out) { SSW_HIP_CHECK(hipMemcpyAsync(coef_out, y, n * plane * sizeof(float), hipMemcpyDeviceToDevice, st)); untimed_work(ctx); }
             if (k_eff == 0) return SSW_OK;
-            SSW_TRY(topk(ctx, st, *sel, y, n, w, h, c.ordering, k_eff, idx));
+            SSW_TRY(topk(ctx, st, *sel, y, n, w, h, c.ordering, k_eff, idx, mask));
             StageTimer t(ctx, SSW_STAGE_EMBED, st);
             return launch_embed(st, y, n, plane, idx, k_eff, marks, nullptr, nullptr, 1, k_eff, k, c.method, c.alpha);
         }});
diff --git a/spread_spectrum_watermarking_amd/csrc/tuning.hip b/spread_spectrum_watermarking_amd/csrc/tuning.hip
--- a/spread_spectrum_watermarking_amd/csrc/tuning.hip
+++ b/spread_spectrum_watermarking_amd/csrc/tuning.hip
@@ -37,6 +37,8 @@
     {"tile48", "SSW_TILE48", 1},
     {"base_prune", "SSW_BASE_PRUNE", 1},
     {"base_energy_lowp", "SSW_BASE_ENERGY_LOWP", 1},
+    {"phase2_jobs", "SSW_PHASE2_JOBS", 1},
+    {"writer_mask", "SSW_WRITER_MASK", 1},
 };
 
 std::mutex g_tune_lock;
```

Result: no change. 17970, median of 6 (+1.1%).
